# facebookresearch/SONAR

Measured on NVIDIA H100. Metric: sentences/sec->1024-d, higher is better.
Workload: dtype bf16

## Files before the change

include/sonar_b200.h:

```cpp
#ifndef SONAR_B200_H_
#define SONAR_B200_H_

#include <stddef.h>
#include <stdint.h>

#ifdef __cplusplus
extern "C" {
#endif

#define SB_OK 0
#define SB_ERR_INVALID (-1)
#define SB_ERR_CUDA (-2)
#define SB_ERR_DRIVER (-3)
#define SB_ERR_INPUT (-4)

#define SB_POOL_MAX 1
#define SB_POOL_MEAN 2
#define SB_POOL_LAST 3
#define SB_POOL_ATTENTION 4

#define SB_EPI_BIAS 0
#define SB_EPI_BIAS_RELU 1
#define SB_EPI_BIAS_RESIDUAL 2
#define SB_EPI_BIAS_SILU 5
#define SB_EPI_BIAS_TANH 7

typedef struct SbEncoder SbEncoder;

typedef struct SbEncoderConfig {
  int32_t model_dim;
  int32_t num_layers;
  int32_t num_heads;
  int32_t ffn_inner_dim;
  int64_t vocab_size;
  int32_t pos_rows;
  int32_t pooling;
  float ln_eps;
  float embed_scale;
  int32_t cta_group;
  int32_t num_sms;
  int32_t ln_fold;
  int32_t embedding_dim;
  int32_t pooler_layers;
  int32_t pooler_heads;
  int32_t pooler_ffn_inner_dim;
} SbEncoderConfig;

typedef struct SbLayerWeights {
  const void* wqkv;
  const float* bqkv;
  const void* wo;
  const float* bo;
  const void* w1;
  const float* b1;
  const void* w2;
  const float* b2;
  const float* ln1_g;
  const float* ln1_b;
  const float* ln2_g;
  const float* ln2_b;
} SbLayerWeights;

typedef struct SbEncoderWeights {
  const void* embed;
  const float* pos_table;
  const float* final_ln_g;
  const float* final_ln_b;
  const SbLayerWeights* layers;
  const float* pooler_q0;
  const void* proj_w;
  const float* proj_b;
  const struct SbPoolerLayerWeights* pooler;
} SbEncoderWeights;

const char* sb_last_error(void);
int sb_version(void);

int sb_encoder_create(const SbEncoderConfig* cfg, const SbEncoderWeights* w, SbEncoder** out);
void sb_encoder_destroy(SbEncoder* enc);

int sb_encoder_workspace_bytes(const SbEncoder* enc, int32_t max_batch, int64_t max_tokens, size_t* bytes);

int sb_encoder_forward(SbEncoder* enc, const int64_t* ids, int64_t ids_row_stride, const int32_t* seq_lens_host,
                       int32_t batch, int32_t seq_len, float* out, float* encoded, void* workspace,
                       size_t workspace_bytes, void* stream);

int sb_encoder_forward_host(SbEncoder* enc, const int64_t* ids_host, const int32_t* seq_lens_host, int32_t batch,
                            int32_t seq_len, float* out_host, int64_t* ids_staging, float* out_staging,
                            void* workspace, size_t workspace_bytes, void* stream);

int sb_encoder_profile_ffn1(SbEncoder* enc, void* start_event, void* stop_event);

int sb_encoder_check_inputs(SbEncoder* enc, void* workspace, void* stream);


int sb_fold_layernorm(const void* W, const float* bias, const float* gamma, const float* beta, int32_t N, int32_t K,
                      void* Wf, float* colsum, float* bias_f, void* stream);
int sb_gemm_ln_consumer(const void* A, int64_t lda, const void* Wf, int64_t ldw, void* C, int64_t ldc, const float* bias_f,
                        const float* colsum, const float* stats, float eps, int32_t M, int32_t N, int32_t K, int32_t relu,
                        void* stream);
int sb_gemm_residual_stats(const void* A, int64_t lda, const void* W, int64_t ldw, float* x, int64_t ldx, const float* bias,
                           void* h_out, int64_t ldh, float* stats_out, int32_t M, int32_t N, int32_t K, void* stream);

int sb_gemm_residual_splitk(const void* A, int64_t lda, const void* W, int64_t ldw, float* x, int64_t ldx, const float* bias,
                            int32_t M, int32_t N, int32_t K, int32_t* counters, int64_t n_counters, void* stream);

int sb_gemm_bf16(const void* A, int64_t lda, const void* W, int64_t ldw, void* C, int64_t ldc, int32_t out_fp32,
                 const float* bias, const void* residual, int64_t ldr, int32_t M, int32_t N, int32_t K, int32_t epi,
                 int32_t cta_group, void* stream);

int sb_layernorm(const float* x, const float* gamma, const float* beta, float eps, void* y, int64_t T, int32_t D,
                 void* stream);

int sb_attention(const void* qkv, const int32_t* cu_seqlens, int32_t B, int32_t H, int64_t total_tokens, void* out,
                 void* stream);

int sb_embed(const int64_t* ids, int64_t ids_row_stride, const int32_t* cu_seqlens, int32_t B, int32_t S,
             const void* embed, int64_t vocab, const float* pos_table, int32_t pos_rows, int32_t D, float scale,
             float* x, int32_t* err_flag, void* stream);

int sb_pool(const float* x, const int32_t* cu_seqlens, int32_t B, int32_t D, const float* gamma, const float* beta,
            float eps, int32_t apply_ln, int32_t pool_mode, float* out, float* encoded_padded, int32_t S_padded,
            void* stream);

int sb_pool_latent_attention(const void* qt, const void* mem, const int32_t* cu_seqlens, int32_t B, int32_t Hd, int32_t D,
                             void* u, void* stream);

int sb_attention_relpos(const void* qkv, const void* p, const float* u_bias, const float* v_bias, const int32_t* cu_seqlens,
                        int32_t B, int32_t H, int64_t total_tokens, int32_t Npad, int32_t S_center, int32_t impl, void* qu,
                        void* qv, float* vp, void* out, void* stream);
int sb_conformer_conv(const void* g, const int32_t* cu_seqlens, int32_t B, int32_t max_len, int32_t D, const float* dw,
                      const float* bn_scale, const float* bn_shift, void* out, void* stream);
int sb_speech_frontend(const float* fbank, int32_t padded_frames, const int32_t* cu_seqlens, int32_t B, int32_t max_len,
                       const float* gamma, const float* beta, float eps, void* out, void* stream);

typedef struct SbDecoder SbDecoder;

typedef struct SbDecoderConfig {
  int32_t model_dim;
  int32_t num_layers;
  int32_t num_heads;
  int32_t ffn_inner_dim;
  int32_t input_dim;
  int64_t vocab_size;
  int32_t pos_rows;
  int32_t eos_idx;
  float ln_eps;
  float embed_scale;
} SbDecoderConfig;

typedef struct SbDecoderLayerWeights {
  const void* wqkv;
  const float* bqkv;
  const void* wo;
  const float* bo;
  const void* cross_wv;
  const float* cross_bv;
  const void* cross_wo;
  const float* cross_bo;
  const void* w1;
  const float* b1;
  const void* w2;
  const float* b2;
  const float* ln1_g;
  const float* ln1_b;
  const float* ln3_g;
  const float* ln3_b;
} SbDecoderLayerWeights;

typedef struct SbDecoderWeights {
  const void* embed;
  const float* pos_table;
  const float* final_ln_g;
  const float* final_ln_b;
  const SbDecoderLayerWeights* layers;
} SbDecoderWeights;

int sb_decoder_create(const SbDecoderConfig* cfg, const SbDecoderWeights* w, SbDecoder** out);
void sb_decoder_destroy(SbDecoder* dec);
int sb_decoder_workspace_bytes(const SbDecoder* dec, int32_t num_sentences, int32_t beam, int32_t max_len, size_t* bytes);
int sb_decoder_begin(SbDecoder* dec, const float* embeddings, int32_t num_sentences, int32_t beam, int32_t max_len,
                     void* workspace, size_t workspace_bytes, void* stream);
int sb_decoder_step(SbDecoder* dec, const int64_t* tokens, const int32_t* table, int32_t t, int32_t num_sentences,
                    int32_t beam, int32_t max_len, float* out_lprob, int32_t* out_tok, float* out_eos_lprob,
                    const int64_t* probe_tokens, float* out_probe_lprob, void* workspace, size_t workspace_bytes,
                    void* stream);
int sb_decoder_check_inputs(SbDecoder* dec, void* workspace, void* stream);

size_t sb_fbank_tables_bytes(void);
int sb_fbank_build_tables(void* host_buf);
int sb_fbank(const float* waves, const int64_t* wave_offsets, const int32_t* frame_offsets, int32_t B,
             int32_t total_frames, const void* tables, float* raw_out, float* out, int32_t padded_frames, void* stream);

typedef struct SbSpeechEncoder SbSpeechEncoder;

typedef struct SbSpeechConfig {
  int32_t model_dim;
  int32_t num_layers;
  int32_t num_heads;
  int32_t ffn_inner_dim;
  int32_t conv_kernel;
  int32_t pooler_layers;
  int32_t pooler_ffn_inner_dim;
  float ln_eps;
  int32_t attn_impl;
} SbSpeechConfig;

typedef struct SbConformerLayerWeights {
  const float* ffn1_ln_g; const float* ffn1_ln_b;
  const void* ffn1_w1; const float* ffn1_b1; const void* ffn1_w2 ; const float* ffn1_b2 ;
  const float* attn_ln_g; const float* attn_ln_b;
  const void* wqkv; const float* bqkv; const void* wo; const float* bo;
  const void* wr;
  const float* u_bias;
  const float* v_bias;
  const float* conv_ln_g; const float* conv_ln_b;
  const void* pw1;
  const float* dw;
  const float* bn_scale;
  const float* bn_shift;
  const void* pw2;
  const float* ffn2_ln_g; const float* ffn2_ln_b;
  const void* ffn2_w1; const float* ffn2_b1; const void* ffn2_w2 ; const float* ffn2_b2 ;
  const float* ln_g; const float* ln_b;
} SbConformerLayerWeights;

typedef struct SbPoolerLayerWeights {
  const void* sa_wv; const float* sa_bv; const void* sa_wo; const float* sa_bo;
  const float* sa_ln_g; const float* sa_ln_b;
  const void* ca_wq; const float* ca_bq;
  const void* ca_wkv ; const float* ca_bkv;
  const void* ca_wo; const float* ca_bo;
  const float* ca_ln_g; const float* ca_ln_b;
  const void* w1; const float* b1; const void* w2; const float* b2;
  const float* ffn_ln_g; const float* ffn_ln_b;
} SbPoolerLayerWeights;

typedef struct SbSpeechWeights {
  const float* front_ln_g;
  const float* front_ln_b;
  const void* front_w;
  const float* front_b;
  const float* final_ln_g;
  const float* final_ln_b;
  const float* pooler_q0;
  const void* proj_w;
  const float* zeros;
  const SbConformerLayerWeights* layers;
  const SbPoolerLayerWeights* pooler;
} SbSpeechWeights;

int sb_speech_encoder_create(const SbSpeechConfig* cfg, const SbSpeechWeights* w, SbSpeechEncoder** out);
void sb_speech_encoder_destroy(SbSpeechEncoder* enc);
int sb_speech_encoder_workspace_bytes(const SbSpeechEncoder* enc, int32_t batch, int64_t total_positions,
                                      int32_t max_positions, size_t* bytes);
int sb_speech_encoder_forward(SbSpeechEncoder* enc, const float* fbank, int32_t padded_frames, const int32_t* cu_dev,
                              const int32_t* lens_host, int32_t batch, const void* relpos_table, int32_t relpos_rows,
                              float* out, float* encoded_packed, void* workspace, size_t workspace_bytes, void* stream);


int sb_xsim_workspace_bytes(int32_t n, int32_t m, int32_t d, size_t* bytes);

int sb_xsim_knn(const float* x, const float* y, int32_t n, int32_t m, int32_t d, int32_t k, double* out_val,
                int32_t* out_idx, void* workspace, size_t workspace_bytes, void* stream);

int sb_xsim_bidir_workspace_bytes(int32_t n, int32_t m, int32_t d, size_t* bytes);
int sb_xsim_knn_bidir(const float* x, const float* y, int32_t n, int32_t m, int32_t d, int32_t k, double* val_xy,
                      int32_t* idx_xy, double* val_yx, int32_t* idx_yx, int32_t* overflow_flag, void* workspace,
                      size_t workspace_bytes, void* stream);

int sb_xsim_margin_predict(const double* val_xy, const int32_t* idx_xy, const double* val_yx, int32_t n, int32_t m,
                           int32_t k, int32_t margin_mode, int32_t* pred, void* stream);

int sb_beam_step(const float* lp, const int32_t* tok, const float* eos_lp, int64_t* seqs, int32_t* table,
                 int64_t* tokens, float* cum, uint8_t* alive, uint8_t* done, float* fin_score, int64_t* fin_seq,
                 int64_t* fin_len, int64_t* fin_count, int32_t N, int32_t beam, int32_t Tmax, int32_t t, int32_t g,
                 int32_t eos_block, int32_t max_gen, int64_t vocab, int32_t eos, int32_t unk, int32_t pad,
                 float unk_penalty, float score_div, int32_t normalize, void* stream);

typedef struct SbLaser2 SbLaser2;

typedef struct SbLaser2Config {
  int64_t vocab_size;
  int64_t pad_idx;
  int32_t embed_dim;
  int32_t hidden_size;
  int32_t num_layers;
  int32_t bidirectional;
  float padding_value;
  int32_t num_sms;
} SbLaser2Config;

typedef struct SbLstmLayerWeights {
  const void* w_ih;
  const void* w_hh;
  const float* b_ih;
  const float* b_hh;
} SbLstmLayerWeights;

typedef struct SbLaser2Weights {
  const void* embed;
  const SbLstmLayerWeights* layers;
} SbLaser2Weights;

int sb_laser2_create(const SbLaser2Config* cfg, const SbLaser2Weights* w, SbLaser2** out);
void sb_laser2_destroy(SbLaser2* enc);
int sb_laser2_workspace_bytes(const SbLaser2* enc, int32_t max_batch, int64_t max_tokens, size_t* bytes);
int sb_laser2_forward(SbLaser2* enc, const int64_t* ids, int64_t ids_row_stride, const int32_t* seq_lens_host, int32_t batch,
                      int32_t seq_len, float* out, void* workspace, size_t workspace_bytes, void* stream);
int sb_laser2_check_inputs(SbLaser2* enc, void* stream);

int sb_lstm_recurrent(const void* G, int64_t ldg, const void* w_hh, const int32_t* cu_seqlens, const int32_t* tile_seqs,
                      int32_t num_tiles, int32_t num_dirs, void* y, int64_t ldy, float* pool_out, int64_t ldp,
                      const uint8_t* pad_mask, const uint8_t* tail_keep, float padding_value, void* stream);

#define SB_BLASER_COMET 0
#define SB_BLASER_QE 1

typedef struct SbBlaser SbBlaser;

typedef struct SbBlaserConfig {
  int32_t input_form;
  int32_t embedding_dim;
  int32_t num_hidden;
  const int32_t* hidden_dims;
  int32_t cta_group;
  int32_t num_sms;
} SbBlaserConfig;

typedef struct SbBlaserWeights {
  const void* const* w;
  const float* const* b;
} SbBlaserWeights;

int sb_blaser_create(const SbBlaserConfig* cfg, const SbBlaserWeights* w, SbBlaser** out);
void sb_blaser_destroy(SbBlaser* model);
int sb_blaser_workspace_bytes(const SbBlaser* model, int32_t max_rows, size_t* bytes);
int sb_blaser_forward(SbBlaser* model, const float* src, const float* mt, const float* ref, int64_t ld, int32_t rows,
                      float* scores, void* workspace, size_t workspace_bytes, void* stream);
int sb_blaser_featurize(const float* src, const float* mt, const float* ref, int64_t ld, int32_t rows, int32_t E,
                        int32_t input_form, int32_t normalize, void* out, int32_t out_fp32, void* stream);

#ifdef __cplusplus
}
#endif
#endif
```

sonar_b200/_lib.py:

```python

from __future__ import annotations

import ctypes as C
from pathlib import Path
from typing import Optional

_LIB_PATH = Path(__file__).resolve().parent / "lib" / "libsonar_b200.so"
_lib: Optional[C.CDLL] = None

SB_POOL_MAX, SB_POOL_MEAN, SB_POOL_LAST, SB_POOL_ATTENTION = 1, 2, 3, 4
SB_EPI_BIAS, SB_EPI_BIAS_RELU, SB_EPI_BIAS_RESIDUAL, SB_EPI_BIAS_TANH = 0, 1, 2, 7
SB_BLASER_COMET, SB_BLASER_QE = 0, 1
SB_ERR_INVALID, SB_ERR_CUDA, SB_ERR_DRIVER, SB_ERR_INPUT = -1, -2, -3, -4


class SbEncoderConfig(C.Structure):
    _fields_ = [
        ("model_dim", C.c_int32), ("num_layers", C.c_int32), ("num_heads", C.c_int32),
        ("ffn_inner_dim", C.c_int32), ("vocab_size", C.c_int64), ("pos_rows", C.c_int32),
        ("pooling", C.c_int32), ("ln_eps", C.c_float), ("embed_scale", C.c_float),
        ("cta_group", C.c_int32), ("num_sms", C.c_int32), ("ln_fold", C.c_int32),
        ("embedding_dim", C.c_int32), ("pooler_layers", C.c_int32), ("pooler_heads", C.c_int32),
        ("pooler_ffn_inner_dim", C.c_int32),
    ]


class SbLayerWeights(C.Structure):
    _fields_ = [(n, C.c_void_p) for n in (
        "wqkv", "bqkv", "wo", "bo", "w1", "b1", "w2", "b2", "ln1_g", "ln1_b", "ln2_g", "ln2_b")]


class SbPoolerLayerWeights(C.Structure):
    _fields_ = [(n, C.c_void_p) for n in (
        "sa_wv", "sa_bv", "sa_wo", "sa_bo", "sa_ln_g", "sa_ln_b", "ca_wq", "ca_bq", "ca_wkv", "ca_bkv", "ca_wo", "ca_bo",
        "ca_ln_g", "ca_ln_b", "w1", "b1", "w2", "b2", "ffn_ln_g", "ffn_ln_b")]


class SbEncoderWeights(C.Structure):
    _fields_ = [("embed", C.c_void_p), ("pos_table", C.c_void_p), ("final_ln_g", C.c_void_p),
                ("final_ln_b", C.c_void_p), ("layers", C.POINTER(SbLayerWeights)),
                ("pooler_q0", C.c_void_p), ("proj_w", C.c_void_p), ("proj_b", C.c_void_p),
                ("pooler", C.POINTER(SbPoolerLayerWeights))]


class SbDecoderConfig(C.Structure):
    _fields_ = [
        ("model_dim", C.c_int32), ("num_layers", C.c_int32), ("num_heads", C.c_int32),
        ("ffn_inner_dim", C.c_int32), ("input_dim", C.c_int32), ("vocab_size", C.c_int64),
        ("pos_rows", C.c_int32), ("eos_idx", C.c_int32), ("ln_eps", C.c_float), ("embed_scale", C.c_float),
    ]


class SbDecoderLayerWeights(C.Structure):
    _fields_ = [(n, C.c_void_p) for n in (
        "wqkv", "bqkv", "wo", "bo", "cross_wv", "cross_bv", "cross_wo", "cross_bo", "w1", "b1", "w2", "b2",
        "ln1_g", "ln1_b", "ln3_g", "ln3_b")]


class SbDecoderWeights(C.Structure):
    _fields_ = [("embed", C.c_void_p), ("pos_table", C.c_void_p), ("final_ln_g", C.c_void_p),
                ("final_ln_b", C.c_void_p), ("layers", C.POINTER(SbDecoderLayerWeights))]


class SbSpeechConfig(C.Structure):
    _fields_ = [("model_dim", C.c_int32), ("num_layers", C.c_int32), ("num_heads", C.c_int32),
                ("ffn_inner_dim", C.c_int32), ("conv_kernel", C.c_int32), ("pooler_layers", C.c_int32),
                ("pooler_ffn_inner_dim", C.c_int32), ("ln_eps", C.c_float), ("attn_impl", C.c_int32)]


class SbConformerLayerWeights(C.Structure):
    _fields_ = [(n, C.c_void_p) for n in (
        "ffn1_ln_g", "ffn1_ln_b", "ffn1_w1", "ffn1_b1", "ffn1_w2", "ffn1_b2", "attn_ln_g", "attn_ln_b", "wqkv", "bqkv",
        "wo", "bo", "wr", "u_bias", "v_bias", "conv_ln_g", "conv_ln_b", "pw1", "dw", "bn_scale", "bn_shift", "pw2",
        "ffn2_ln_g", "ffn2_ln_b", "ffn2_w1", "ffn2_b1", "ffn2_w2", "ffn2_b2", "ln_g", "ln_b")]


class SbSpeechWeights(C.Structure):
    _fields_ = [(n, C.c_void_p) for n in ("front_ln_g", "front_ln_b", "front_w", "front_b", "final_ln_g", "final_ln_b",
                                          "pooler_q0", "proj_w", "zeros")] + \
               [("layers", C.POINTER(SbConformerLayerWeights)), ("pooler", C.POINTER(SbPoolerLayerWeights))]


class SbLaser2Config(C.Structure):
    _fields_ = [("vocab_size", C.c_int64), ("pad_idx", C.c_int64), ("embed_dim", C.c_int32), ("hidden_size", C.c_int32),
                ("num_layers", C.c_int32), ("bidirectional", C.c_int32), ("padding_value", C.c_float),
                ("num_sms", C.c_int32)]


class SbLstmLayerWeights(C.Structure):
    _fields_ = [(n, C.c_void_p) for n in ("w_ih", "w_hh", "b_ih", "b_hh")]


class SbLaser2Weights(C.Structure):
    _fields_ = [("embed", C.c_void_p), ("layers", C.POINTER(SbLstmLayerWeights))]


class SbBlaserConfig(C.Structure):
    _fields_ = [("input_form", C.c_int32), ("embedding_dim", C.c_int32), ("num_hidden", C.c_int32),
                ("hidden_dims", C.POINTER(C.c_int32)), ("cta_group", C.c_int32), ("num_sms", C.c_int32)]


class SbBlaserWeights(C.Structure):
    _fields_ = [("w", C.POINTER(C.c_void_p)), ("b", C.POINTER(C.c_void_p))]


_SIGNATURES = {
    "sb_last_error": (C.c_char_p, []),
    "sb_version": (C.c_int, []),
    "sb_encoder_create": (C.c_int, [C.POINTER(SbEncoderConfig), C.POINTER(SbEncoderWeights),
                                    C.POINTER(C.c_void_p)]),
    "sb_encoder_destroy": (None, [C.c_void_p]),
    "sb_encoder_workspace_bytes": (C.c_int, [C.c_void_p, C.c_int32, C.c_int64, C.POINTER(C.c_size_t)]),
    "sb_encoder_forward": (C.c_int, [C.c_void_p, C.c_void_p, C.c_int64, C.c_void_p, C.c_int32, C.c_int32,
                                     C.c_void_p, C.c_void_p, C.c_void_p, C.c_size_t, C.c_void_p]),
    "sb_encoder_forward_host": (C.c_int, [C.c_void_p, C.c_void_p, C.c_void_p, C.c_int32, C.c_int32,
                                          C.c_void_p, C.c_void_p, C.c_void_p, C.c_void_p, C.c_size_t,
                                          C.c_void_p]),
    "sb_encoder_profile_ffn1": (C.c_int, [C.c_void_p, C.c_void_p, C.c_void_p]),
    "sb_encoder_check_inputs": (C.c_int, [C.c_void_p, C.c_void_p, C.c_void_p]),
    "sb_gemm_bf16": (C.c_int, [C.c_void_p, C.c_int64, C.c_void_p, C.c_int64, C.c_void_p, C.c_int64,
                               C.c_int32, C.c_void_p, C.c_void_p, C.c_int64, C.c_int32, C.c_int32,
                               C.c_int32, C.c_int32, C.c_int32, C.c_void_p]),
    "sb_layernorm": (C.c_int, [C.c_void_p, C.c_void_p, C.c_void_p, C.c_float, C.c_void_p, C.c_int64,
                               C.c_int32, C.c_void_p]),
    "sb_attention": (C.c_int, [C.c_void_p, C.c_void_p, C.c_int32, C.c_int32, C.c_int64, C.c_void_p, C.c_void_p]),
    "sb_embed": (C.c_int, [C.c_void_p, C.c_int64, C.c_void_p, C.c_int32, C.c_int32, C.c_void_p, C.c_int64,
                           C.c_void_p, C.c_int32, C.c_int32, C.c_float, C.c_void_p, C.c_void_p, C.c_void_p]),
    "sb_pool": (C.c_int, [C.c_void_p, C.c_void_p, C.c_int32, C.c_int32, C.c_void_p, C.c_void_p, C.c_float,
                          C.c_int32, C.c_int32, C.c_void_p, C.c_void_p, C.c_int32, C.c_void_p]),
    "sb_pool_latent_attention": (C.c_int, [C.c_void_p, C.c_void_p, C.c_void_p, C.c_int32, C.c_int32, C.c_int32,
                                           C.c_void_p, C.c_void_p]),
    "sb_attention_relpos": (C.c_int, [C.c_void_p] * 5 + [C.c_int32, C.c_int32, C.c_int64, C.c_int32, C.c_int32, C.c_int32] +
                            [C.c_void_p] * 5),
    "sb_conformer_conv": (C.c_int, [C.c_void_p, C.c_void_p, C.c_int32, C.c_int32, C.c_int32] + [C.c_void_p] * 5),
    "sb_speech_frontend": (C.c_int, [C.c_void_p, C.c_int32, C.c_void_p, C.c_int32, C.c_int32, C.c_void_p, C.c_void_p,
                                     C.c_float, C.c_void_p, C.c_void_p]),
    "sb_decoder_create": (C.c_int, [C.POINTER(SbDecoderConfig), C.POINTER(SbDecoderWeights), C.POINTER(C.c_void_p)]),
    "sb_decoder_destroy": (None, [C.c_void_p]),
    "sb_decoder_workspace_bytes": (C.c_int, [C.c_void_p, C.c_int32, C.c_int32, C.c_int32, C.POINTER(C.c_size_t)]),
    "sb_decoder_begin": (C.c_int, [C.c_void_p, C.c_void_p, C.c_int32, C.c_int32, C.c_int32, C.c_void_p, C.c_size_t,
                                   C.c_void_p]),
    "sb_decoder_step": (C.c_int, [C.c_void_p, C.c_void_p, C.c_void_p, C.c_int32, C.c_int32, C.c_int32, C.c_int32,
                                  C.c_void_p, C.c_void_p, C.c_void_p, C.c_void_p, C.c_void_p, C.c_void_p, C.c_size_t,
                                  C.c_void_p]),
    "sb_decoder_check_inputs": (C.c_int, [C.c_void_p, C.c_void_p, C.c_void_p]),
    "sb_fbank_tables_bytes": (C.c_size_t, []),
    "sb_fbank_build_tables": (C.c_int, [C.c_void_p]),
    "sb_fbank": (C.c_int, [C.c_void_p, C.c_void_p, C.c_void_p, C.c_int32, C.c_int32, C.c_void_p, C.c_void_p,
                           C.c_void_p, C.c_int32, C.c_void_p]),
    "sb_speech_encoder_create": (C.c_int, [C.POINTER(SbSpeechConfig), C.POINTER(SbSpeechWeights), C.POINTER(C.c_void_p)]),
    "sb_speech_encoder_destroy": (None, [C.c_void_p]),
    "sb_speech_encoder_workspace_bytes": (C.c_int, [C.c_void_p, C.c_int32, C.c_int64, C.c_int32, C.POINTER(C.c_size_t)]),
    "sb_speech_encoder_forward": (C.c_int, [C.c_void_p, C.c_void_p, C.c_int32, C.c_void_p, C.c_void_p, C.c_int32,
                                            C.c_void_p, C.c_int32, C.c_void_p, C.c_void_p, C.c_void_p, C.c_size_t,
                                            C.c_void_p]),
    "sb_xsim_workspace_bytes": (C.c_int, [C.c_int32, C.c_int32, C.c_int32, C.POINTER(C.c_size_t)]),
    "sb_xsim_knn": (C.c_int, [C.c_void_p, C.c_void_p, C.c_int32, C.c_int32, C.c_int32, C.c_int32, C.c_void_p,
                              C.c_void_p, C.c_void_p, C.c_size_t, C.c_void_p]),
    "sb_xsim_margin_predict": (C.c_int, [C.c_void_p, C.c_void_p, C.c_void_p, C.c_int32, C.c_int32, C.c_int32,
                                         C.c_int32, C.c_void_p, C.c_void_p]),
    "sb_fold_layernorm": (C.c_int, [C.c_void_p] * 4 + [C.c_int32, C.c_int32] + [C.c_void_p] * 4),
    "sb_gemm_ln_consumer": (C.c_int, [C.c_void_p, C.c_int64, C.c_void_p, C.c_int64, C.c_void_p, C.c_int64, C.c_void_p,
                                      C.c_void_p, C.c_void_p, C.c_float, C.c_int32, C.c_int32, C.c_int32, C.c_int32,
                                      C.c_void_p]),
    "sb_gemm_residual_stats": (C.c_int, [C.c_void_p, C.c_int64, C.c_void_p, C.c_int64, C.c_void_p, C.c_int64, C.c_void_p,
                                         C.c_void_p, C.c_int64, C.c_void_p, C.c_int32, C.c_int32, C.c_int32, C.c_void_p]),
    "sb_gemm_residual_splitk": (C.c_int, [C.c_void_p, C.c_int64, C.c_void_p, C.c_int64, C.c_void_p, C.c_int64, C.c_void_p,
                                          C.c_int32, C.c_int32, C.c_int32, C.c_void_p, C.c_int64, C.c_void_p]),
    "sb_xsim_bidir_workspace_bytes": (C.c_int, [C.c_int32, C.c_int32, C.c_int32, C.POINTER(C.c_size_t)]),
    "sb_xsim_knn_bidir": (C.c_int, [C.c_void_p, C.c_void_p, C.c_int32, C.c_int32, C.c_int32, C.c_int32, C.c_void_p, C.c_void_p,
                                    C.c_void_p, C.c_void_p, C.c_void_p, C.c_void_p, C.c_size_t, C.c_void_p]),
    "sb_beam_step": (C.c_int, [C.c_void_p] * 13 + [C.c_int32] * 7 + [C.c_int64] + [C.c_int32] * 3 +
                     [C.c_float, C.c_float, C.c_int32, C.c_void_p]),
    "sb_laser2_create": (C.c_int, [C.POINTER(SbLaser2Config), C.POINTER(SbLaser2Weights), C.POINTER(C.c_void_p)]),
    "sb_laser2_destroy": (None, [C.c_void_p]),
    "sb_laser2_workspace_bytes": (C.c_int, [C.c_void_p, C.c_int32, C.c_int64, C.POINTER(C.c_size_t)]),
    "sb_laser2_forward": (C.c_int, [C.c_void_p, C.c_void_p, C.c_int64, C.c_void_p, C.c_int32, C.c_int32, C.c_void_p,
                                    C.c_void_p, C.c_size_t, C.c_void_p]),
    "sb_laser2_check_inputs": (C.c_int, [C.c_void_p, C.c_void_p]),
    "sb_lstm_recurrent": (C.c_int, [C.c_void_p, C.c_int64, C.c_void_p, C.c_void_p, C.c_void_p, C.c_int32, C.c_int32,
                                    C.c_void_p, C.c_int64, C.c_void_p, C.c_int64, C.c_void_p, C.c_void_p, C.c_float,
                                    C.c_void_p]),
    "sb_blaser_create": (C.c_int, [C.POINTER(SbBlaserConfig), C.POINTER(SbBlaserWeights), C.POINTER(C.c_void_p)]),
    "sb_blaser_destroy": (None, [C.c_void_p]),
    "sb_blaser_workspace_bytes": (C.c_int, [C.c_void_p, C.c_int32, C.POINTER(C.c_size_t)]),
    "sb_blaser_forward": (C.c_int, [C.c_void_p, C.c_void_p, C.c_void_p, C.c_void_p, C.c_int64, C.c_int32, C.c_void_p,
                                    C.c_void_p, C.c_size_t, C.c_void_p]),
    "sb_blaser_featurize": (C.c_int, [C.c_void_p, C.c_void_p, C.c_void_p, C.c_int64, C.c_int32, C.c_int32, C.c_int32,
                                      C.c_int32, C.c_void_p, C.c_int32, C.c_void_p]),
}


def lib_path() -> Path:
    return _LIB_PATH


def load() -> C.CDLL:
    global _lib
    if _lib is not None:
        return _lib
    if not _LIB_PATH.exists():
        raise RuntimeError(
            f"sonar_b200: native library {_LIB_PATH} is missing -- run `python -m sonar_b200.build` "
            "(or `__graft_entry__.build()`); there is no CPU/PyTorch fallback path.")
    lib = C.CDLL(str(_LIB_PATH))
    for name, (restype, argtypes) in _SIGNATURES.items():
        fn = getattr(lib, name)
        fn.restype = restype
        fn.argtypes = argtypes
    _lib = lib
    return lib


def last_error() -> str:
    msg = load().sb_last_error()
    return msg.decode("utf-8", "replace") if msg else ""


def workspace_bytes(query, *args) -> int:
    need = C.c_size_t()
    check(query(*args, C.byref(need)), query.__name__)
    return need.value


def check(rc: int, what: str) -> None:
    if rc == 0:
        return
    msg = f"{what}: {last_error()} (code {rc})"
    if rc in (SB_ERR_INVALID, SB_ERR_INPUT):
        raise ValueError(msg)
    raise RuntimeError(msg)
```

sonar_b200/csrc/common.cuh:

```cuda
#pragma once

#include <cuda.h>
#include <cuda_bf16.h>
#include <cuda_runtime.h>
#include <stdint.h>
#include <stdio.h>

namespace sb {

void set_last_error(const char* fmt, ...);

#define SB_CUDA_CHECK(expr)                                                              \
  do {                                                                                   \
    cudaError_t _e = (expr);                                                             \
    if (_e != cudaSuccess) {                                                             \
      ::sb::set_last_error("%s failed: %s (%s:%d)", #expr, cudaGetErrorString(_e),       \
                           __FILE__, __LINE__);                                          \
      return -2;                                                                         \
    }                                                                                    \
  } while (0)

__device__ __forceinline__ uint32_t smem_u32(const void* p) {
  return static_cast<uint32_t>(__cvta_generic_to_shared(p));
}

__device__ __forceinline__ uint32_t lane_id() {
  uint32_t l;
  asm volatile("mov.u32 %0, %%laneid;" : "=r"(l));
  return l;
}

__device__ __forceinline__ uint32_t cluster_ctarank() {
  uint32_t r;
  asm volatile("mov.u32 %0, %%cluster_ctarank;" : "=r"(r));
  return r;
}

__device__ __forceinline__ bool elect_one() {
  uint32_t pred = 0;
  asm volatile(
      "{\n\t"
      ".reg .pred p;\n\t"
      "elect.sync _|p, 0xffffffff;\n\t"
      "selp.u32 %0, 1, 0, p;\n\t"
      "}\n"
      : "=r"(pred));
  return pred != 0;
}

__device__ __forceinline__ void cluster_sync_all() {
  asm volatile("barrier.cluster.arrive.release.aligned;\n\t"
               "barrier.cluster.wait.acquire.aligned;\n" ::: "memory");
}

__device__ __forceinline__ void named_bar_sync(uint32_t id, uint32_t nthreads) {
  asm volatile("bar.sync %0, %1;" ::"r"(id), "r"(nthreads) : "memory");
}

__device__ __forceinline__ void mbar_init(uint64_t* bar, uint32_t count) {
  asm volatile("mbarrier.init.shared::cta.b64 [%0], %1;" ::"r"(smem_u32(bar)), "r"(count) : "memory");
}

__device__ __forceinline__ void fence_mbar_init() {
  asm volatile("fence.mbarrier_init.release.cluster;" ::: "memory");
}

__device__ __forceinline__ void mbar_arrive_expect_tx(uint64_t* bar, uint32_t bytes) {
  asm volatile("mbarrier.arrive.expect_tx.shared::cta.b64 _, [%0], %1;" ::"r"(smem_u32(bar)), "r"(bytes)
               : "memory");
}

__device__ __forceinline__ void mbar_arrive(uint64_t* bar) {
  asm volatile("mbarrier.arrive.shared::cta.b64 _, [%0];" ::"r"(smem_u32(bar)) : "memory");
}

__device__ __forceinline__ void mbar_arrive_cluster(uint64_t* bar, uint32_t cta) {
  asm volatile(
      "{\n\t"
      ".reg .b32 ra;\n\t"
      "mapa.shared::cluster.u32 ra, %0, %1;\n\t"
      "mbarrier.arrive.shared::cluster.b64 _, [ra];\n\t"
      "}\n" ::"r"(smem_u32(bar)),
      "r"(cta)
      : "memory");
}

__device__ __forceinline__ bool mbar_try_wait(uint64_t* bar, uint32_t parity) {
  uint32_t ok;
  asm volatile(
      "{\n\t"
      ".reg .pred p;\n\t"
      "mbarrier.try_wait.parity.shared::cta.b64 p, [%1], %2;\n\t"
      "selp.u32 %0, 1, 0, p;\n\t"
      "}\n"
      : "=r"(ok)
      : "r"(smem_u32(bar)), "r"(parity)
      : "memory");
  return ok != 0;
}

__device__ __forceinline__ bool mbar_test_wait(uint64_t* bar, uint32_t parity) {
  uint32_t ok;
  asm volatile(
      "{\n\t"
      ".reg .pred p;\n\t"
      "mbarrier.test_wait.parity.shared::cta.b64 p, [%1], %2;\n\t"
      "selp.u32 %0, 1, 0, p;\n\t"
      "}\n"
      : "=r"(ok)
      : "r"(smem_u32(bar)), "r"(parity)
      : "memory");
  return ok != 0;
}

#ifndef SB_MBAR_TIMEOUT_CYCLES
#define SB_MBAR_TIMEOUT_CYCLES (4000000000ll)
#endif
__device__ __forceinline__ void mbar_wait(uint64_t* bar, uint32_t parity) {
  if (mbar_try_wait(bar, parity)) return;
  const long long t0 = clock64();
  while (!mbar_try_wait(bar, parity)) {
    if (clock64() - t0 > SB_MBAR_TIMEOUT_CYCLES) __trap();
  }
}

__device__ __forceinline__ void tma_prefetch_desc(const CUtensorMap* m) {
  asm volatile("prefetch.tensormap [%0];" ::"l"(reinterpret_cast<uint64_t>(m)) : "memory");
}

__device__ __forceinline__ void tma_load_2d(void* smem_dst, const CUtensorMap* m, uint64_t* bar, int c0,
                                            int c1) {
  asm volatile(
      "cp.async.bulk.tensor.2d.shared::cluster.global.mbarrier::complete_tx::bytes [%0], [%1, {%3, %4}], [%2];" ::"r"(
          smem_u32(smem_dst)),
      "l"(reinterpret_cast<uint64_t>(m)), "r"(smem_u32(bar)), "r"(c0), "r"(c1)
      : "memory");
}

__device__ __forceinline__ void tma_load_2d_multicast(void* smem_dst, const CUtensorMap* m, uint64_t* bar, int c0, int c1,
                                                      uint16_t cta_mask) {
  asm volatile(
      "cp.async.bulk.tensor.2d.shared::cluster.global.mbarrier::complete_tx::bytes.multicast::cluster [%0], [%1, {%3, "
      "%4}], [%2], %5;" ::"r"(smem_u32(smem_dst)),
      "l"(reinterpret_cast<uint64_t>(m)), "r"(smem_u32(bar)), "r"(c0), "r"(c1), "h"(cta_mask)
      : "memory");
}

__device__ __forceinline__ void tma_store_2d(const CUtensorMap* m, const void* smem_src, int c0, int c1) {
  asm volatile("cp.async.bulk.tensor.2d.global.shared::cta.bulk_group [%0, {%2, %3}], [%1];" ::"l"(
                   reinterpret_cast<uint64_t>(m)),
               "r"(smem_u32(smem_src)), "r"(c0), "r"(c1)
               : "memory");
}

__device__ __forceinline__ void tma_reduce_add_2d(const CUtensorMap* m, const void* smem_src, int c0, int c1) {
  asm volatile("cp.reduce.async.bulk.tensor.2d.global.shared::cta.add.bulk_group [%0, {%2, %3}], [%1];" ::"l"(
                   reinterpret_cast<uint64_t>(m)),
               "r"(smem_u32(smem_src)), "r"(c0), "r"(c1)
               : "memory");
}

__device__ __forceinline__ void tma_store_commit() { asm volatile("cp.async.bulk.commit_group;" ::: "memory"); }

template <int N>
__device__ __forceinline__ void tma_store_wait_read() {
  asm volatile("cp.async.bulk.wait_group.read %0;" ::"n"(N) : "memory");
}

template <int N>
__device__ __forceinline__ void tma_store_wait_all() {
  asm volatile("cp.async.bulk.wait_group %0;" ::"n"(N) : "memory");
}

__device__ __forceinline__ void fence_proxy_async_all() { asm volatile("fence.proxy.async;" ::: "memory"); }
__device__ __forceinline__ int ld_acquire_gpu(const int* p) {
  int v;
  asm volatile("ld.acquire.gpu.global.s32 %0, [%1];" : "=r"(v) : "l"(p) : "memory");
  return v;
}
__device__ __forceinline__ void st_release_gpu(int* p, int v) {
  asm volatile("st.release.gpu.global.s32 [%0], %1;" ::"l"(p), "r"(v) : "memory");
}

__device__ __forceinline__ void fence_proxy_async_smem() {
  asm volatile("fence.proxy.async.shared::cta;" ::: "memory");
}

__device__ __forceinline__ void stmatrix_x4(uint32_t smem_addr, uint32_t r0, uint32_t r1, uint32_t r2, uint32_t r3) {
  asm volatile("stmatrix.sync.aligned.m8n8.x4.shared.b16 [%0], {%1, %2, %3, %4};" ::"r"(smem_addr), "r"(r0), "r"(r1),
               "r"(r2), "r"(r3)
               : "memory");
}

__device__ __forceinline__ void st_shared_v2(uint32_t smem_addr, float x, float y) {
  asm volatile("st.shared.v2.f32 [%0], {%1, %2};" ::"r"(smem_addr), "f"(x), "f"(y) : "memory");
}

__device__ __forceinline__ void wgmma_fence() { asm volatile("wgmma.fence.sync.aligned;" ::: "memory"); }
__device__ __forceinline__ void wgmma_commit() { asm volatile("wgmma.commit_group.sync.aligned;" ::: "memory"); }
template <int N>
__device__ __forceinline__ void wgmma_wait() {
  asm volatile("wgmma.wait_group.sync.aligned %0;" ::"n"(N) : "memory");
}
template <int N>
__device__ __forceinline__ void wgmma_fence_regs(float (&d)[N]) {
#pragma unroll
  for (int i = 0; i < N; ++i) asm volatile("" : "+f"(d[i])::"memory");
}

template <int kRegs>
__device__ __forceinline__ void setmaxnreg_inc() {
  asm volatile("setmaxnreg.inc.sync.aligned.u32 %0;" ::"n"(kRegs));
}
template <int kRegs>
__device__ __forceinline__ void setmaxnreg_dec() {
  asm volatile("setmaxnreg.dec.sync.aligned.u32 %0;" ::"n"(kRegs));
}

__device__ __forceinline__ uint64_t wgmma_desc_kmajor_sw128(uint32_t smem_addr) {
  return uint64_t((smem_addr >> 4) & 0x3FFFu)
         | (uint64_t(1024u >> 4) << 32)
         | (uint64_t(1) << 62);
}
__device__ __forceinline__ uint64_t wgmma_desc_mnmajor_sw128(uint32_t smem_addr) {
  return uint64_t((smem_addr >> 4) & 0x3FFFu) | (uint64_t(1) << 16) | (uint64_t(1024u >> 4) << 32) | (uint64_t(1) << 62);
}

__device__ __forceinline__ void wgmma_m64n256k16_ss(float (&d)[128], uint64_t a_desc, uint64_t b_desc, uint32_t accumulate) {
  asm volatile(
      "{\n\t"
      ".reg .pred p;\n\t"
      "setp.ne.b32 p, %130, 0;\n\t"
      "wgmma.mma_async.sync.aligned.m64n256k16.f32.bf16.bf16 {"
      "%0, %1, %2, %3, %4, %5, %6, %7, %8, %9, %10, %11, %12, %13, %14, %15, %16, %17, %18, %19, %20, %21, %22, %23, "
      "%24, %25, %26, %27, %28, %29, %30, %31, %32, %33, %34, %35, %36, %37, %38, %39, %40, %41, %42, %43, %44, %45, "
      "%46, %47, %48, %49, %50, %51, %52, %53, %54, %55, %56, %57, %58, %59, %60, %61, %62, %63, %64, %65, %66, %67, "
      "%68, %69, %70, %71, %72, %73, %74, %75, %76, %77, %78, %79, %80, %81, %82, %83, %84, %85, %86, %87, %88, %89, "
      "%90, %91, %92, %93, %94, %95, %96, %97, %98, %99, %100, %101, %102, %103, %104, %105, %106, %107, %108, %109, "
      "%110, %111, %112, %113, %114, %115, %116, %117, %118, %119, %120, %121, %122, %123, %124, %125, %126, %127"
      "}, %128, %129, p, 1, 1, 0, 0;\n\t"
      "}\n"
      : "+f"(d[0]), "+f"(d[1]), "+f"(d[2]), "+f"(d[3]), "+f"(d[4]), "+f"(d[5]), "+f"(d[6]), "+f"(d[7]),
        "+f"(d[8]), "+f"(d[9]), "+f"(d[10]), "+f"(d[11]), "+f"(d[12]), "+f"(d[13]), "+f"(d[14]), "+f"(d[15]),
        "+f"(d[16]), "+f"(d[17]), "+f"(d[18]), "+f"(d[19]), "+f"(d[20]), "+f"(d[21]), "+f"(d[22]), "+f"(d[23]),
        "+f"(d[24]), "+f"(d[25]), "+f"(d[26]), "+f"(d[27]), "+f"(d[28]), "+f"(d[29]), "+f"(d[30]), "+f"(d[31]),
        "+f"(d[32]), "+f"(d[33]), "+f"(d[34]), "+f"(d[35]), "+f"(d[36]), "+f"(d[37]), "+f"(d[38]), "+f"(d[39]),
        "+f"(d[40]), "+f"(d[41]), "+f"(d[42]), "+f"(d[43]), "+f"(d[44]), "+f"(d[45]), "+f"(d[46]), "+f"(d[47]),
        "+f"(d[48]), "+f"(d[49]), "+f"(d[50]), "+f"(d[51]), "+f"(d[52]), "+f"(d[53]), "+f"(d[54]), "+f"(d[55]),
        "+f"(d[56]), "+f"(d[57]), "+f"(d[58]), "+f"(d[59]), "+f"(d[60]), "+f"(d[61]), "+f"(d[62]), "+f"(d[63]),
        "+f"(d[64]), "+f"(d[65]), "+f"(d[66]), "+f"(d[67]), "+f"(d[68]), "+f"(d[69]), "+f"(d[70]), "+f"(d[71]),
        "+f"(d[72]), "+f"(d[73]), "+f"(d[74]), "+f"(d[75]), "+f"(d[76]), "+f"(d[77]), "+f"(d[78]), "+f"(d[79]),
        "+f"(d[80]), "+f"(d[81]), "+f"(d[82]), "+f"(d[83]), "+f"(d[84]), "+f"(d[85]), "+f"(d[86]), "+f"(d[87]),
        "+f"(d[88]), "+f"(d[89]), "+f"(d[90]), "+f"(d[91]), "+f"(d[92]), "+f"(d[93]), "+f"(d[94]), "+f"(d[95]),
        "+f"(d[96]), "+f"(d[97]), "+f"(d[98]), "+f"(d[99]), "+f"(d[100]), "+f"(d[101]), "+f"(d[102]), "+f"(d[103]),
        "+f"(d[104]), "+f"(d[105]), "+f"(d[106]), "+f"(d[107]), "+f"(d[108]), "+f"(d[109]), "+f"(d[110]), "+f"(d[111]),
        "+f"(d[112]), "+f"(d[113]), "+f"(d[114]), "+f"(d[115]), "+f"(d[116]), "+f"(d[117]), "+f"(d[118]), "+f"(d[119]),
        "+f"(d[120]), "+f"(d[121]), "+f"(d[122]), "+f"(d[123]), "+f"(d[124]), "+f"(d[125]), "+f"(d[126]), "+f"(d[127])
      : "l"(a_desc), "l"(b_desc), "r"(accumulate));
}

__device__ __forceinline__ void wgmma_m64n128k16_ss(float (&d)[64], uint64_t a_desc, uint64_t b_desc, uint32_t accumulate) {
  asm volatile(
      "{\n\t"
      ".reg .pred p;\n\t"
      "setp.ne.b32 p, %66, 0;\n\t"
      "wgmma.mma_async.sync.aligned.m64n128k16.f32.bf16.bf16 {"
      "%0, %1, %2, %3, %4, %5, %6, %7, %8, %9, %10, %11, %12, %13, %14, %15, %16, %17, %18, %19, %20, %21, %22, %23, "
      "%24, %25, %26, %27, %28, %29, %30, %31, %32, %33, %34, %35, %36, %37, %38, %39, %40, %41, %42, %43, %44, %45, "
      "%46, %47, %48, %49, %50, %51, %52, %53, %54, %55, %56, %57, %58, %59, %60, %61, %62, %63"
      "}, %64, %65, p, 1, 1, 0, 0;\n\t"
      "}\n"
      : "+f"(d[0]), "+f"(d[1]), "+f"(d[2]), "+f"(d[3]), "+f"(d[4]), "+f"(d[5]), "+f"(d[6]), "+f"(d[7]),
        "+f"(d[8]), "+f"(d[9]), "+f"(d[10]), "+f"(d[11]), "+f"(d[12]), "+f"(d[13]), "+f"(d[14]), "+f"(d[15]),
        "+f"(d[16]), "+f"(d[17]), "+f"(d[18]), "+f"(d[19]), "+f"(d[20]), "+f"(d[21]), "+f"(d[22]), "+f"(d[23]),
        "+f"(d[24]), "+f"(d[25]), "+f"(d[26]), "+f"(d[27]), "+f"(d[28]), "+f"(d[29]), "+f"(d[30]), "+f"(d[31]),
        "+f"(d[32]), "+f"(d[33]), "+f"(d[34]), "+f"(d[35]), "+f"(d[36]), "+f"(d[37]), "+f"(d[38]), "+f"(d[39]),
        "+f"(d[40]), "+f"(d[41]), "+f"(d[42]), "+f"(d[43]), "+f"(d[44]), "+f"(d[45]), "+f"(d[46]), "+f"(d[47]),
        "+f"(d[48]), "+f"(d[49]), "+f"(d[50]), "+f"(d[51]), "+f"(d[52]), "+f"(d[53]), "+f"(d[54]), "+f"(d[55]),
        "+f"(d[56]), "+f"(d[57]), "+f"(d[58]), "+f"(d[59]), "+f"(d[60]), "+f"(d[61]), "+f"(d[62]), "+f"(d[63])
      : "l"(a_desc), "l"(b_desc), "r"(accumulate));
}

__device__ __forceinline__ void wgmma_m64n96k16_ss(float (&d)[48], uint64_t a_desc, uint64_t b_desc, uint32_t accumulate) {
  asm volatile(
      "{\n\t"
      ".reg .pred p;\n\t"
      "setp.ne.b32 p, %50, 0;\n\t"
      "wgmma.mma_async.sync.aligned.m64n96k16.f32.bf16.bf16 {"
      "%0, %1, %2, %3, %4, %5, %6, %7, %8, %9, %10, %11, %12, %13, %14, %15, %16, %17, %18, %19, %20, %21, %22, %23, "
      "%24, %25, %26, %27, %28, %29, %30, %31, %32, %33, %34, %35, %36, %37, %38, %39, %40, %41, %42, %43, %44, %45, "
      "%46, %47"
      "}, %48, %49, p, 1, 1, 0, 0;\n\t"
      "}\n"
      : "+f"(d[0]), "+f"(d[1]), "+f"(d[2]), "+f"(d[3]), "+f"(d[4]), "+f"(d[5]), "+f"(d[6]), "+f"(d[7]),
        "+f"(d[8]), "+f"(d[9]), "+f"(d[10]), "+f"(d[11]), "+f"(d[12]), "+f"(d[13]), "+f"(d[14]), "+f"(d[15]),
        "+f"(d[16]), "+f"(d[17]), "+f"(d[18]), "+f"(d[19]), "+f"(d[20]), "+f"(d[21]), "+f"(d[22]), "+f"(d[23]),
        "+f"(d[24]), "+f"(d[25]), "+f"(d[26]), "+f"(d[27]), "+f"(d[28]), "+f"(d[29]), "+f"(d[30]), "+f"(d[31]),
        "+f"(d[32]), "+f"(d[33]), "+f"(d[34]), "+f"(d[35]), "+f"(d[36]), "+f"(d[37]), "+f"(d[38]), "+f"(d[39]),
        "+f"(d[40]), "+f"(d[41]), "+f"(d[42]), "+f"(d[43]), "+f"(d[44]), "+f"(d[45]), "+f"(d[46]), "+f"(d[47])
      : "l"(a_desc), "l"(b_desc), "r"(accumulate));
}

__device__ __forceinline__ void wgmma_m64n64k16_rs_bt(float (&d)[32], const uint32_t (&a)[4], uint64_t b_desc, uint32_t accumulate) {
  asm volatile(
      "{\n\t"
      ".reg .pred p;\n\t"
      "setp.ne.b32 p, %37, 0;\n\t"
      "wgmma.mma_async.sync.aligned.m64n64k16.f32.bf16.bf16 {"
      "%0, %1, %2, %3, %4, %5, %6, %7, %8, %9, %10, %11, %12, %13, %14, %15, %16, %17, %18, %19, %20, %21, %22, %23, "
      "%24, %25, %26, %27, %28, %29, %30, %31"
      "}, {%32, %33, %34, %35}, %36, p, 1, 1, 1;\n\t"
      "}\n"
      : "+f"(d[0]), "+f"(d[1]), "+f"(d[2]), "+f"(d[3]), "+f"(d[4]), "+f"(d[5]), "+f"(d[6]), "+f"(d[7]),
        "+f"(d[8]), "+f"(d[9]), "+f"(d[10]), "+f"(d[11]), "+f"(d[12]), "+f"(d[13]), "+f"(d[14]), "+f"(d[15]),
        "+f"(d[16]), "+f"(d[17]), "+f"(d[18]), "+f"(d[19]), "+f"(d[20]), "+f"(d[21]), "+f"(d[22]), "+f"(d[23]),
        "+f"(d[24]), "+f"(d[25]), "+f"(d[26]), "+f"(d[27]), "+f"(d[28]), "+f"(d[29]), "+f"(d[30]), "+f"(d[31])
      : "r"(a[0]), "r"(a[1]), "r"(a[2]), "r"(a[3]), "l"(b_desc), "r"(accumulate));
}

__device__ __forceinline__ void mma_m16n8k16_bf16(float (&d)[4], const uint32_t (&a)[4], uint32_t b0, uint32_t b1) {
  asm volatile("mma.sync.aligned.m16n8k16.row.col.f32.bf16.bf16.f32 {%0,%1,%2,%3}, {%4,%5,%6,%7}, {%8,%9}, {%0,%1,%2,%3};"
               : "+f"(d[0]), "+f"(d[1]), "+f"(d[2]), "+f"(d[3])
               : "r"(a[0]), "r"(a[1]), "r"(a[2]), "r"(a[3]), "r"(b0), "r"(b1));
}

__device__ __forceinline__ float ex2_approx(float x) {
  float y;
  asm("ex2.approx.ftz.f32 %0, %1;" : "=f"(y) : "f"(x));
  return y;
}

__device__ __forceinline__ uint32_t pack_bf16x2(float lo, float hi) {
  __nv_bfloat162 v = __floats2bfloat162_rn(lo, hi);
  return *reinterpret_cast<uint32_t*>(&v);
}

__device__ __forceinline__ float warp_sum(float v) {
#pragma unroll
  for (int o = 16; o > 0; o >>= 1) v += __shfl_xor_sync(0xffffffffu, v, o);
  return v;
}
__device__ __forceinline__ float warp_max(float v) {
#pragma unroll
  for (int o = 16; o > 0; o >>= 1) v = fmaxf(v, __shfl_xor_sync(0xffffffffu, v, o));
  return v;
}

}

namespace sb {
static constexpr int kMaxVec = 8;

template <bool kL2 = false>
__device__ __forceinline__ void load_row(const float* row, int nvec, int lane, float4 (&v)[kMaxVec]) {
#pragma unroll
  for (int i = 0; i < kMaxVec; ++i)
    if (i < nvec) v[i] = kL2 ? __ldcg(reinterpret_cast<const float4*>(row + (i * 32 + lane) * 4))
                        : *reinterpret_cast<const float4*>(row + (i * 32 + lane) * 4);
}

__device__ __forceinline__ void normalize_row(float4 (&v)[kMaxVec], int nvec, int lane, int D,
                                              const float* __restrict__ gamma, const float* __restrict__ beta,
                                              float eps) {
  float s = 0.f;
#pragma unroll
  for (int i = 0; i < kMaxVec; ++i)
    if (i < nvec) s += (v[i].x + v[i].y) + (v[i].z + v[i].w);
  const float mean = warp_sum(s) / float(D);
  float q = 0.f;
#pragma unroll
  for (int i = 0; i < kMaxVec; ++i)
    if (i < nvec) {
      const float a = v[i].x - mean, b = v[i].y - mean, c = v[i].z - mean, d = v[i].w - mean;
      q += (a * a + b * b) + (c * c + d * d);
    }
  const float rstd = 1.0f / sqrtf(warp_sum(q) / float(D) + eps);
#pragma unroll
  for (int i = 0; i < kMaxVec; ++i)
    if (i < nvec) {
      const float4 g = __ldg(reinterpret_cast<const float4*>(gamma) + i * 32 + lane);
      const float4 bt = __ldg(reinterpret_cast<const float4*>(beta) + i * 32 + lane);
      v[i].x = (v[i].x - mean) * rstd * g.x + bt.x;
      v[i].y = (v[i].y - mean) * rstd * g.y + bt.y;
      v[i].z = (v[i].z - mean) * rstd * g.z + bt.z;
      v[i].w = (v[i].w - mean) * rstd * g.w + bt.w;
    }
}

}

__device__ __forceinline__ float tanh_approx(float x) {
  float y;
  asm("tanh.approx.f32 %0, %1;" : "=f"(y) : "f"(x));
  return y;
}
__device__ __forceinline__ float sigmoid_fast(float x) { return fmaf(0.5f, tanh_approx(0.5f * x), 0.5f); }
__device__ __forceinline__ float silu_fast(float x) {
  const float h = 0.5f * x;
  return fmaf(h, tanh_approx(h), h);
}
```

sonar_b200/csrc/encoder.cu:

```cuda

#include "../../include/sonar_b200.h"
#include <stdlib.h>

#include "common.cuh"
#include "sonar_b200_internal.h"

#include <cstdarg>
#include <cstdio>
#include <cstring>
#include <new>
#include <vector>

namespace sb {

static thread_local char g_err[512] = "";

void set_last_error(const char* fmt, ...) {
  va_list ap;
  va_start(ap, fmt);
  vsnprintf(g_err, sizeof(g_err), fmt, ap);
  va_end(ap);
}

int require_hopper(const char* who, int* num_sms) {
  int n_gpu = 0, dev = 0, major = 0, minor = 0;
  if (cudaGetDeviceCount(&n_gpu) != cudaSuccess || n_gpu == 0) {
    set_last_error("%s: no CUDA device (this engine has no CPU path)", who);
    return SB_ERR_CUDA;
  }
  SB_CUDA_CHECK(cudaGetDevice(&dev));
  SB_CUDA_CHECK(cudaDeviceGetAttribute(&major, cudaDevAttrComputeCapabilityMajor, dev));
  SB_CUDA_CHECK(cudaDeviceGetAttribute(&minor, cudaDevAttrComputeCapabilityMinor, dev));
  if (major != 9) {
    set_last_error("%s: the sm_90a kernels need a Hopper H100-class GPU (found sm_%d%d)", who, major, minor);
    return SB_ERR_CUDA;
  }
  SB_CUDA_CHECK(cudaDeviceGetAttribute(num_sms, cudaDevAttrMultiProcessorCount, dev));
  return SB_OK;
}

struct Workspace {
  int32_t* cu;
  float* ln_stats;
  float* x;
  __nv_bfloat16* h;
  __nv_bfloat16* qkv;
  __nv_bfloat16* f;
  AttentionPooler::Ws pool;
  size_t bytes;
};

}

using namespace sb;

struct FoldedLayer {
  __nv_bfloat16* wqkv = nullptr;
  __nv_bfloat16* w1 = nullptr;
  float* cqkv = nullptr;
  float* bqkv = nullptr;
  float* c1 = nullptr;
  float* b1 = nullptr;
};

struct SbEncoder {
  SbEncoderConfig cfg;
  int out_dim;
  std::vector<FoldedLayer> folded;
  void* fold_pool = nullptr;
  int32_t* err_flag = nullptr;
  const void* embed;
  const float* pos_table;
  const float* final_ln_g;
  const float* final_ln_b;
  std::vector<SbLayerWeights> layers;
  AttentionPooler pooler;
  int num_sms;
  static constexpr int kSlots = 8;
  static constexpr int kSlotInts = 32768 + 8;
  int32_t* pinned = nullptr;
  cudaEvent_t ev[kSlots];
  bool ev_ok[kSlots];
  unsigned next_slot = 0;
  cudaEvent_t prof_start = nullptr, prof_stop = nullptr;
};

static Workspace carve(const SbEncoder* e, int32_t max_batch, int64_t max_tokens, void* base) {
  const size_t D = e->cfg.model_dim, F = e->cfg.ffn_inner_dim;
  const size_t T = (size_t)(max_tokens > 0 ? max_tokens : 1);
  Carver c(base);
  Workspace w;
  w.cu = c.take<int32_t>(sizeof(int32_t) * ((size_t)max_batch + 1));
  w.ln_stats = c.take<float>(T * (D / kLnPartCols) * 2 * sizeof(float));
  w.x = c.take<float>(T * D * 4);
  w.h = c.take<__nv_bfloat16>(T * D * 2);
  w.qkv = c.take<__nv_bfloat16>(T * 3 * D * 2);
  w.f = c.take<__nv_bfloat16>(T * F * 2);
  w.pool = {};
  if (e->cfg.pooling == SB_POOL_ATTENTION) w.pool = e->pooler.take(c, (size_t)max_batch);
  w.bytes = c.off;
  return w;
}

extern "C" {

const char* sb_last_error(void) { return g_err; }
int sb_version(void) { return 109; }

int sb_encoder_create(const SbEncoderConfig* cfg, const SbEncoderWeights* w, SbEncoder** out) {
  if (!cfg || !w || !out) { set_last_error("sb_encoder_create: null argument"); return SB_ERR_INVALID; }
  *out = nullptr;
  const int D = cfg->model_dim, H = cfg->num_heads, F = cfg->ffn_inner_dim;
  if (D <= 0 || D % 256 != 0 || D > 1024) {
    set_last_error("sb_encoder_create: model_dim must be a multiple of 256 and <= 1024 (got %d)", D);
    return SB_ERR_INVALID;
  }
  if (H <= 0 || D != H * 64) {
    set_last_error("sb_encoder_create: head_dim must be 64 (model_dim=%d, num_heads=%d)", D, H);
    return SB_ERR_INVALID;
  }
  if (F <= 0 || F % 256 != 0) { set_last_error("sb_encoder_create: ffn_inner_dim must be a multiple of 256"); return SB_ERR_INVALID; }
  if (cfg->ln_fold < 0 || cfg->ln_fold > 2) { set_last_error("sb_encoder_create: ln_fold must be 0, 1 or 2"); return SB_ERR_INVALID; }
  if (cfg->num_layers < 0 || cfg->pos_rows <= 0 || cfg->vocab_size <= 0) {
    set_last_error("sb_encoder_create: bad num_layers / pos_rows / vocab_size");
    return SB_ERR_INVALID;
  }
  const bool attn_pool = cfg->pooling == SB_POOL_ATTENTION;
  if (cfg->pooling != SB_POOL_MAX && cfg->pooling != SB_POOL_MEAN && cfg->pooling != SB_POOL_LAST && !attn_pool) {
    set_last_error("sb_encoder_create: unsupported pooling %d", cfg->pooling);
    return SB_ERR_INVALID;
  }
  const int E = cfg->embedding_dim;
  if (attn_pool) {
    if (E <= 0 || E % 256 != 0 || E > 1024 || E != 64 * cfg->pooler_heads) {
      set_last_error("sb_encoder_create: attention pooling needs embedding_dim = 64 * pooler_heads, a multiple of 256 and "
                     "<= 1024 (embedding_dim=%d, pooler_heads=%d)", E, cfg->pooler_heads);
      return SB_ERR_INVALID;
    }
    if (cfg->pooler_ffn_inner_dim <= 0 || cfg->pooler_ffn_inner_dim % 256 != 0 || cfg->pooler_layers < 1) {
      set_last_error("sb_encoder_create: attention pooling needs pooler_layers >= 1 and pooler_ffn_inner_dim a multiple of 256 "
                     "(got %d, %d)", cfg->pooler_layers, cfg->pooler_ffn_inner_dim);
      return SB_ERR_INVALID;
    }
  } else if (E != 0 && E != D) {
    set_last_error("sb_encoder_create: embedding_dim (%d) != model_dim (%d) needs attention pooling", E, D);
    return SB_ERR_INVALID;
  }
  if (!w->embed || !w->pos_table || !w->final_ln_g || !w->final_ln_b || (cfg->num_layers > 0 && !w->layers)) {
    set_last_error("sb_encoder_create: missing weight pointer");
    return SB_ERR_INVALID;
  }
  for (int i = 0; i < cfg->num_layers; ++i)
    if (has_null_pointer(w->layers[i])) {
      set_last_error("sb_encoder_create: layer %d has a null weight pointer", i);
      return SB_ERR_INVALID;
    }
  int num_sms = 0;
  if (int rc = require_hopper("sb_encoder_create", &num_sms)) return rc;
  SbEncoder* e = new (std::nothrow) SbEncoder();
  if (!e) { set_last_error("out of host memory"); return SB_ERR_INVALID; }
  e->cfg = *cfg;
  e->embed = w->embed;
  e->pos_table = w->pos_table;
  e->final_ln_g = w->final_ln_g;
  e->final_ln_b = w->final_ln_b;
  e->layers.assign(w->layers, w->layers + cfg->num_layers);
  e->out_dim = attn_pool ? E : D;
  e->num_sms = cfg->num_sms > 0 ? cfg->num_sms : num_sms;
  for (int i = 0; i < SbEncoder::kSlots; ++i) e->ev_ok[i] = false;
  if (cudaMallocHost(reinterpret_cast<void**>(&e->pinned), sizeof(int32_t) * SbEncoder::kSlots * SbEncoder::kSlotInts) !=
      cudaSuccess) {
    set_last_error("sb_encoder_create: cudaMallocHost failed");
    delete e;
    return SB_ERR_CUDA;
  }
  if (cudaMalloc(reinterpret_cast<void**>(&e->err_flag), 256) != cudaSuccess ||
      cudaMemset(e->err_flag, 0, 256) != cudaSuccess) {
    set_last_error("sb_encoder_create: cudaMalloc of the input-check flag failed");
    sb_encoder_destroy(e);
    return SB_ERR_CUDA;
  }
  if (cfg->ln_fold && cfg->num_layers > 0) {
    const size_t D_ = D, F_ = F;
    auto carve_folded = [&](void* base) {
      Carver c(base);
      for (FoldedLayer& f : e->folded) {
        f.wqkv = c.take<__nv_bfloat16>(3 * D_ * D_ * 2, 256);
        f.w1 = c.take<__nv_bfloat16>(F_ * D_ * 2, 256);
        f.cqkv = c.take<float>(3 * D_ * 4, 256);
        f.bqkv = c.take<float>(3 * D_ * 4, 256);
        f.c1 = c.take<float>(F_ * 4, 256);
        f.b1 = c.take<float>(F_ * 4, 256);
      }
      return c.off;
    };
    e->folded.resize(cfg->num_layers);
    const size_t pool_bytes = carve_folded(nullptr);
    if (cudaMalloc(&e->fold_pool, pool_bytes) != cudaSuccess) {
      set_last_error("sb_encoder_create: cudaMalloc of %zu bytes for the LayerNorm-folded weights failed", pool_bytes);
      sb_encoder_destroy(e);
      return SB_ERR_CUDA;
    }
    carve_folded(e->fold_pool);
    for (int i = 0; i < cfg->num_layers; ++i) {
      const FoldedLayer& f = e->folded[i];
      const SbLayerWeights& l = e->layers[i];
      int rc = fold_layernorm_weights(reinterpret_cast<const __nv_bfloat16*>(l.wqkv), l.bqkv, l.ln1_g, l.ln1_b, 3 * D, D,
                                      f.wqkv, f.cqkv, f.bqkv, nullptr);
      if (!rc)
        rc = fold_layernorm_weights(reinterpret_cast<const __nv_bfloat16*>(l.w1), l.b1, l.ln2_g, l.ln2_b, F, D, f.w1, f.c1,
                                    f.b1, nullptr);
      if (rc) { sb_encoder_destroy(e); return rc; }
    }
    if (cudaDeviceSynchronize() != cudaSuccess) {
      set_last_error("sb_encoder_create: folding the LayerNorm weights failed: %s", cudaGetErrorString(cudaGetLastError()));
      sb_encoder_destroy(e);
      return SB_ERR_CUDA;
    }
  }
  if (attn_pool) {
    const int rc = e->pooler.create("sb_encoder_create", w->pooler, cfg->pooler_layers, w->pooler_q0, w->proj_w, w->proj_b,
                                    D, E, cfg->pooler_ffn_inner_dim, cfg->ln_eps, e->num_sms, cfg->cta_group == 1 ? 1 : 2, 0);
    if (rc) { sb_encoder_destroy(e); return rc; }
  }
  for (int i = 0; i < SbEncoder::kSlots; ++i) {
    if (cudaEventCreateWithFlags(&e->ev[i], cudaEventDisableTiming) != cudaSuccess) {
      set_last_error("sb_encoder_create: cudaEventCreate failed");
      sb_encoder_destroy(e);
      return SB_ERR_CUDA;
    }
    e->ev_ok[i] = true;
  }
  *out = e;
  return SB_OK;
}

void sb_encoder_destroy(SbEncoder* e) {
  if (!e) return;
  for (int i = 0; i < SbEncoder::kSlots; ++i)
    if (e->ev_ok[i]) cudaEventDestroy(e->ev[i]);
  if (e->pinned) cudaFreeHost(e->pinned);
  if (e->fold_pool) cudaFree(e->fold_pool);
  e->pooler.destroy();
  if (e->err_flag) cudaFree(e->err_flag);
  delete e;
}

int sb_encoder_workspace_bytes(const SbEncoder* enc, int32_t max_batch, int64_t max_tokens, size_t* bytes) {
  if (!enc || !bytes || max_batch <= 0 || max_tokens <= 0) {
    set_last_error("sb_encoder_workspace_bytes: bad argument");
    return SB_ERR_INVALID;
  }
  *bytes = carve(enc, max_batch, max_tokens, nullptr).bytes + kWorkspaceAlign;
  return SB_OK;
}

int sb_encoder_forward(SbEncoder* e, const int64_t* ids, int64_t ids_row_stride, const int32_t* seq_lens_host,
                       int32_t B, int32_t S, float* out, float* encoded, void* workspace, size_t workspace_bytes,
                       void* stream_v) {
  if (!e || !ids || !out || !workspace) { set_last_error("sb_encoder_forward: null argument"); return SB_ERR_INVALID; }
  if (B <= 0 || S <= 0) { set_last_error("sb_encoder_forward: empty batch (B=%d, S=%d)", B, S); return SB_ERR_INVALID; }
  if (S > e->cfg.pos_rows) {
    set_last_error("sb_encoder_forward: seq_len %d exceeds the encoder's max_seq_len %d", S, e->cfg.pos_rows);
    return SB_ERR_INVALID;
  }
  if (B + 1 > SbEncoder::kSlotInts) { set_last_error("sb_encoder_forward: batch too large (%d)", B); return SB_ERR_INVALID; }
  if (ids_row_stride < S) { set_last_error("sb_encoder_forward: ids_row_stride < seq_len"); return SB_ERR_INVALID; }
  cudaStream_t stream = reinterpret_cast<cudaStream_t>(stream_v);
  const int D = e->cfg.model_dim, F = e->cfg.ffn_inner_dim, H = e->cfg.num_heads;

  const unsigned slot = e->next_slot++ % SbEncoder::kSlots;
  SB_CUDA_CHECK(cudaEventSynchronize(e->ev[slot]));
  int32_t* cu_h = e->pinned + (size_t)slot * SbEncoder::kSlotInts;
  long long T = 0;
  cu_h[0] = 0;
  for (int b = 0; b < B; ++b) {
    const int len = seq_lens_host ? seq_lens_host[b] : S;
    if (len < 0 || len > S) { set_last_error("sb_encoder_forward: seq_lens[%d]=%d outside [0,%d]", b, len, S); return SB_ERR_INVALID; }
    T += len;
    if (T > 0x7fffffffll) { set_last_error("sb_encoder_forward: too many tokens"); return SB_ERR_INVALID; }
    cu_h[b + 1] = (int32_t)T;
  }
  Workspace w;
  int rc = bind_workspace("sb_encoder_forward", workspace, workspace_bytes, &w,
                          [&](void* p) { return carve(e, B, T, p); });
  if (rc) return rc;
  SB_CUDA_CHECK(cudaMemcpyAsync(w.cu, cu_h, sizeof(int32_t) * (B + 1), cudaMemcpyHostToDevice, stream));
  SB_CUDA_CHECK(cudaEventRecord(e->ev[slot], stream));
  const bool attn_pool = e->cfg.pooling == SB_POOL_ATTENTION;
  if (T == 0) {
    if (!attn_pool) {
      SB_CUDA_CHECK(cudaMemsetAsync(out, 0, sizeof(float) * (size_t)B * D, stream));
      return SB_OK;
    }
    if (encoded) SB_CUDA_CHECK(cudaMemsetAsync(encoded, 0, sizeof(float) * (size_t)B * S * D, stream));
    return e->pooler.forward(w.pool, w.h, w.cu, B, out, stream);
  }

  const bool fold = e->cfg.ln_fold != 0 && e->cfg.num_layers > 0;
  const bool fold2 = fold && e->cfg.ln_fold == 1;
  __nv_bfloat16* hn = w.qkv;
  if ((rc = embed_tokens(ids, ids_row_stride, w.cu, B, S, reinterpret_cast<const __nv_bfloat16*>(e->embed),
                         e->cfg.vocab_size, e->pos_table, e->cfg.pos_rows, D, e->cfg.embed_scale, w.x, e->err_flag,
                         stream, 0, fold ? w.h : nullptr, fold ? w.ln_stats : nullptr)))
    return rc;

  const int cta_group = (e->cfg.cta_group == 1) ? 1 : 2;
  const int M = (int)T;
  LnFold consume;
  consume.stats_in = w.ln_stats;
  consume.chunks = D / kLnPartCols;
  consume.eps = e->cfg.ln_eps;
  for (int li = 0; li < e->cfg.num_layers; ++li) {
    const SbLayerWeights& L = e->layers[li];
    const FoldedLayer* f = fold ? &e->folded[li] : nullptr;
    if (!fold)
      if ((rc = layernorm_bf16(w.x, L.ln1_g, L.ln1_b, e->cfg.ln_eps, w.h, T, D, stream))) return rc;
    GemmArgs qkv = gemm_args(w.h, D, fold ? f->wqkv : L.wqkv, D, w.qkv, 3 * D, 0, fold ? f->bqkv : L.bqkv, M, 3 * D, D,
                             EPI_BIAS, e->num_sms);
    qkv.cta_group = cta_group;
    if (fold) { qkv.lf = consume; qkv.lf.colsum = f->cqkv; }
    if ((rc = gemm_bf16(qkv, stream))) return rc;
    if ((rc = attention_packed(w.qkv, w.cu, B, H, T, e->num_sms, w.h, stream))) return rc;
    GemmArgs proj = gemm_args(w.h, D, L.wo, D, w.x, D, 1, L.bo, M, D, D, EPI_BIAS_RESIDUAL, e->num_sms);
    proj.cta_group = cta_group;
    if (fold2) {
      proj.epi = EPI_BIAS_RESIDUAL_STATS;
      proj.lf.h_out = hn; proj.lf.ldh = D; proj.lf.stats_out = w.ln_stats;
    }
    if ((rc = gemm_bf16(proj, stream))) return rc;
    if (!fold2)
      if ((rc = layernorm_bf16(w.x, L.ln2_g, L.ln2_b, e->cfg.ln_eps, w.h, T, D, stream))) return rc;
    GemmArgs ffn1 = gemm_args(fold2 ? hn : w.h, D, fold2 ? f->w1 : L.w1, D, w.f, F, 0, fold2 ? f->b1 : L.b1, M, F, D,
                              EPI_BIAS_RELU, e->num_sms);
    ffn1.cta_group = cta_group;
    if (fold2) { ffn1.lf = consume; ffn1.lf.colsum = f->c1; }
    const bool prof = e->prof_start && li == e->cfg.num_layers / 2;
    if (prof) SB_CUDA_CHECK(cudaEventRecord(e->prof_start, stream));
    if ((rc = gemm_bf16(ffn1, stream))) return rc;
    if (prof) SB_CUDA_CHECK(cudaEventRecord(e->prof_stop, stream));
    GemmArgs ffn2 = gemm_args(w.f, F, L.w2, F, w.x, D, 1, L.b2, M, D, F, EPI_BIAS_RESIDUAL, e->num_sms);
    ffn2.cta_group = cta_group;
    if (fold && li + 1 < e->cfg.num_layers) {
      ffn2.epi = EPI_BIAS_RESIDUAL_STATS;
      ffn2.lf.h_out = w.h; ffn2.lf.ldh = D; ffn2.lf.stats_out = w.ln_stats;
    }
    if ((rc = gemm_bf16(ffn2, stream))) return rc;
  }
  if (!attn_pool)
    return ln_pool(w.x, w.cu, B, D, e->final_ln_g, e->final_ln_b, e->cfg.ln_eps, 1, e->cfg.pooling, out, encoded, S,
                   stream);
  if ((rc = layernorm_dual(w.x, e->final_ln_g, e->final_ln_b, e->cfg.ln_eps, w.x, w.h, T, D, stream))) return rc;
  if (encoded)
    if ((rc = ln_pool(w.x, w.cu, B, D, nullptr, nullptr, e->cfg.ln_eps, 0, POOL_LAST, w.pool.px, encoded, S, stream)))
      return rc;
  return e->pooler.forward(w.pool, w.h, w.cu, B, out, stream);
}

int sb_encoder_forward_host(SbEncoder* e, const int64_t* ids_host, const int32_t* seq_lens_host, int32_t B,
                            int32_t S, float* out_host, int64_t* ids_staging, float* out_staging, void* workspace,
                            size_t workspace_bytes, void* stream_v) {
  if (!e || !ids_host || !out_host || !ids_staging || !out_staging) {
    set_last_error("sb_encoder_forward_host: null argument");
    return SB_ERR_INVALID;
  }
  if (B <= 0 || S <= 0) { set_last_error("sb_encoder_forward_host: empty batch"); return SB_ERR_INVALID; }
  cudaStream_t stream = reinterpret_cast<cudaStream_t>(stream_v);
  SB_CUDA_CHECK(cudaMemcpyAsync(ids_staging, ids_host, sizeof(int64_t) * (size_t)B * S, cudaMemcpyHostToDevice, stream));
  int rc = sb_encoder_forward(e, ids_staging, S, seq_lens_host, B, S, out_staging, nullptr, workspace, workspace_bytes,
                              stream_v);
  if (rc) return rc;
  SB_CUDA_CHECK(cudaMemcpyAsync(out_host, out_staging, sizeof(float) * (size_t)B * e->out_dim,
                                cudaMemcpyDeviceToHost, stream));
  SB_CUDA_CHECK(cudaStreamSynchronize(stream));
  return SB_OK;
}

int sb_encoder_profile_ffn1(SbEncoder* e, void* start_event, void* stop_event) {
  if (!e || (!start_event) != (!stop_event)) { set_last_error("sb_encoder_profile_ffn1: bad argument"); return SB_ERR_INVALID; }
  e->prof_start = reinterpret_cast<cudaEvent_t>(start_event);
  e->prof_stop = reinterpret_cast<cudaEvent_t>(stop_event);
  return SB_OK;
}

int sb_encoder_check_inputs(SbEncoder* e, void* workspace, void* stream_v) {
  (void)workspace;
  if (!e) { set_last_error("sb_encoder_check_inputs: null argument"); return SB_ERR_INVALID; }
  cudaStream_t stream = reinterpret_cast<cudaStream_t>(stream_v);
  int32_t flag = 0;
  SB_CUDA_CHECK(cudaMemcpyAsync(&flag, e->err_flag, sizeof(int32_t), cudaMemcpyDeviceToHost, stream));
  SB_CUDA_CHECK(cudaMemsetAsync(e->err_flag, 0, sizeof(int32_t), stream));
  SB_CUDA_CHECK(cudaStreamSynchronize(stream));
  if (flag != 0) {
    set_last_error("token id outside [0, vocab_size) in a batch passed to sb_encoder_forward since the last check");
    return SB_ERR_INPUT;
  }
  return SB_OK;
}

int sb_gemm_bf16(const void* A, int64_t lda, const void* W, int64_t ldw, void* C, int64_t ldc, int32_t out_fp32,
                 const float* bias, const void* residual, int64_t ldr, int32_t M, int32_t N, int32_t K, int32_t epi,
                 int32_t cta_group, void* stream) {
  if (!A || !W || !C) { set_last_error("sb_gemm_bf16: null pointer"); return SB_ERR_INVALID; }
  int sms = 0;
  if (int rc = require_hopper("sb_gemm_bf16", &sms)) return rc;
  GemmArgs g = gemm_args(A, lda, W, ldw, C, ldc, out_fp32, bias, M, N, K, epi, sms);
  g.residual = residual; g.ldr = ldr;
  g.cta_group = cta_group == 1 ? 1 : 2;
  g.allow_skinny = (cta_group == 0);
  return gemm_bf16(g, reinterpret_cast<cudaStream_t>(stream));
}

int sb_fold_layernorm(const void* W, const float* bias, const float* gamma, const float* beta, int32_t N, int32_t K,
                      void* Wf, float* colsum, float* bias_f, void* stream) {
  if (!W || !bias || !gamma || !beta || !Wf || !colsum || !bias_f || N <= 0 || K <= 0) {
    set_last_error("sb_fold_layernorm: bad argument");
    return SB_ERR_INVALID;
  }
  return fold_layernorm_weights(reinterpret_cast<const __nv_bfloat16*>(W), bias, gamma, beta, N, K,
                                reinterpret_cast<__nv_bfloat16*>(Wf), colsum, bias_f, reinterpret_cast<cudaStream_t>(stream));
}

int sb_gemm_ln_consumer(const void* A, int64_t lda, const void* Wf, int64_t ldw, void* C, int64_t ldc, const float* bias_f,
                        const float* colsum, const float* stats, float eps, int32_t M, int32_t N, int32_t K, int32_t relu,
                        void* stream) {
  if (!A || !Wf || !C || !bias_f || !colsum || !stats) { set_last_error("sb_gemm_ln_consumer: null pointer"); return SB_ERR_INVALID; }
  int sms = 0;
  if (int rc = require_hopper("sb_gemm_ln_consumer", &sms)) return rc;
  GemmArgs g = gemm_args(A, lda, Wf, ldw, C, ldc, 0, bias_f, M, N, K, relu ? EPI_BIAS_RELU : EPI_BIAS, sms);
  g.lf.stats_in = stats; g.lf.colsum = colsum; g.lf.chunks = K / kLnPartCols; g.lf.eps = eps;
  return gemm_bf16(g, reinterpret_cast<cudaStream_t>(stream));
}

int sb_gemm_residual_stats(const void* A, int64_t lda, const void* W, int64_t ldw, float* x, int64_t ldx, const float* bias,
                           void* h_out, int64_t ldh, float* stats_out, int32_t M, int32_t N, int32_t K, void* stream) {
  if (!A || !W || !x || !bias || !h_out || !stats_out) { set_last_error("sb_gemm_residual_stats: null pointer"); return SB_ERR_INVALID; }
  int sms = 0;
  if (int rc = require_hopper("sb_gemm_residual_stats", &sms)) return rc;
  GemmArgs g = gemm_args(A, lda, W, ldw, x, ldx, 1, bias, M, N, K, EPI_BIAS_RESIDUAL_STATS, sms);
  g.lf.h_out = reinterpret_cast<__nv_bfloat16*>(h_out); g.lf.ldh = ldh; g.lf.stats_out = stats_out;
  return gemm_bf16(g, reinterpret_cast<cudaStream_t>(stream));
}

int sb_gemm_residual_splitk(const void* A, int64_t lda, const void* W, int64_t ldw, float* x, int64_t ldx, const float* bias,
                            int32_t M, int32_t N, int32_t K, int32_t* counters, int64_t n_counters, void* stream) {
  if (!A || !W || !x || !bias || !counters) { set_last_error("sb_gemm_residual_splitk: null pointer"); return SB_ERR_INVALID; }
  int sms = 0;
  if (int rc = require_hopper("sb_gemm_residual_splitk", &sms)) return rc;
  GemmArgs g = gemm_args(A, lda, W, ldw, x, ldx, 1, bias, M, N, K, EPI_BIAS_RESIDUAL, sms);
  g.splitk_flags = counters;
  g.splitk_flags_len = n_counters;
  return gemm_bf16(g, reinterpret_cast<cudaStream_t>(stream));
}

int sb_layernorm(const float* x, const float* gamma, const float* beta, float eps, void* y, int64_t T, int32_t D,
                 void* stream) {
  if (!x || !gamma || !beta || !y) { set_last_error("sb_layernorm: null pointer"); return SB_ERR_INVALID; }
  return layernorm_bf16(x, gamma, beta, eps, reinterpret_cast<__nv_bfloat16*>(y), T, D,
                        reinterpret_cast<cudaStream_t>(stream));
}

int sb_attention(const void* qkv, const int32_t* cu_seqlens, int32_t B, int32_t H, int64_t total_tokens, void* out,
                 void* stream) {
  if (!qkv || !cu_seqlens || !out) { set_last_error("sb_attention: null pointer"); return SB_ERR_INVALID; }
  int sms = 0;
  if (int rc = require_hopper("sb_attention", &sms)) return rc;
  return attention_packed(reinterpret_cast<const __nv_bfloat16*>(qkv), cu_seqlens, B, H, total_tokens, sms,
                          reinterpret_cast<__nv_bfloat16*>(out), reinterpret_cast<cudaStream_t>(stream));
}

int sb_embed(const int64_t* ids, int64_t ids_row_stride, const int32_t* cu_seqlens, int32_t B, int32_t S,
             const void* embed, int64_t vocab, const float* pos_table, int32_t pos_rows, int32_t D, float scale,
             float* x, int32_t* err_flag, void* stream) {
  if (!ids || !cu_seqlens || !embed || !pos_table || !x || !err_flag) {
    set_last_error("sb_embed: null pointer");
    return SB_ERR_INVALID;
  }
  return embed_tokens(ids, ids_row_stride, cu_seqlens, B, S, reinterpret_cast<const __nv_bfloat16*>(embed), vocab,
                      pos_table, pos_rows, D, scale, x, err_flag, reinterpret_cast<cudaStream_t>(stream));
}

int sb_pool_latent_attention(const void* qt, const void* mem, const int32_t* cu_seqlens, int32_t B, int32_t Hd, int32_t D,
                             void* u, void* stream) {
  if (!qt || !mem || !cu_seqlens || !u) { set_last_error("sb_pool_latent_attention: null pointer"); return SB_ERR_INVALID; }
  int sms = 0;
  if (int rc = require_hopper("sb_pool_latent_attention", &sms)) return rc;
  return pool_latent_attention(reinterpret_cast<const __nv_bfloat16*>(qt), reinterpret_cast<const __nv_bfloat16*>(mem),
                               cu_seqlens, B, Hd, D, reinterpret_cast<__nv_bfloat16*>(u), reinterpret_cast<cudaStream_t>(stream));
}

int sb_pool(const float* x, const int32_t* cu_seqlens, int32_t B, int32_t D, const float* gamma, const float* beta,
            float eps, int32_t apply_ln, int32_t pool_mode, float* out, float* encoded_padded, int32_t S_padded,
            void* stream) {
  if (!x || !cu_seqlens || !out) { set_last_error("sb_pool: null pointer"); return SB_ERR_INVALID; }
  return ln_pool(x, cu_seqlens, B, D, gamma, beta, eps, apply_ln, pool_mode, out, encoded_padded, S_padded,
                 reinterpret_cast<cudaStream_t>(stream));
}

}
```

sonar_b200/csrc/gemm_wgmma.cu:

```cuda

#include "common.cuh"
#include "sonar_b200_internal.h"

#include <math_constants.h>

namespace sb {

constexpr bool epi_row_wise(int epi) { return epi == EPI_BIAS_RESIDUAL_STATS || epi == EPI_TOPK; }

template <int kCtaGroup, int kEpi>
struct GemmCfg {
  static constexpr bool ROW_WISE = epi_row_wise(kEpi);
  static constexpr int BLOCK_M = 128;
  static constexpr int BLOCK_N = 256;
  static constexpr int BLOCK_K = 64;
  static constexpr int LOAD_N = BLOCK_N / kCtaGroup;
  static constexpr int A_BYTES = BLOCK_M * BLOCK_K * 2;
  static constexpr int B_BYTES = BLOCK_N * BLOCK_K * 2;
  static constexpr int STAGES = ROW_WISE ? 3 : 4;
  static constexpr int EPI_GROUPS = 2;
  static constexpr int CD_BYTES = 2 * 64 * 128;
  static constexpr int TRANS_LD = 68;
  static constexpr int TRANS_BYTES = ROW_WISE ? 64 * TRANS_LD * 4 : 0;
  static constexpr int LN_BYTES = 64 * 8;
  static constexpr int BAR_BYTES = 256;
  static constexpr int SMEM_BYTES =
      STAGES * (A_BYTES + B_BYTES) + 2 * (CD_BYTES + TRANS_BYTES + LN_BYTES) + BAR_BYTES + 1024 ;
  static constexpr int THREADS = 384;
  static_assert(SMEM_BYTES <= 232448, "shared memory budget of one sm_90 block");
  static_assert(2 * STAGES * 8 <= BAR_BYTES, "ring barriers");
};

template <bool kSweep>
struct TileSched {
  int num_m_tiles, num_n_tiles, cluster_id, num_clusters, n_chunks, tiles_per_chunk;
  int k_splits = 1;
  int i = 0, j = 0;
  __device__ __forceinline__ bool next(int& m_blk, int& n_blk, int& chunk, bool& first, bool& last) {
    if constexpr (!kSweep) {
      const int item = cluster_id + i * num_clusters;
      ++i;
      const int tiles = num_m_tiles * num_n_tiles;
      if (item >= tiles * k_splits) return false;
      const int tile = (k_splits == 1) ? item : item % tiles;
      chunk = (k_splits == 1) ? 0 : item / tiles;
      m_blk = tile / num_n_tiles;
      n_blk = tile % num_n_tiles;
      first = last = true;
      return true;
    } else {
      for (;;) {
        const int item = cluster_id + i * num_clusters;
        if (item >= num_m_tiles * n_chunks) return false;
        m_blk = item / n_chunks;
        chunk = item % n_chunks;
        const int n_begin = chunk * tiles_per_chunk;
        const int cnt = min(tiles_per_chunk, num_n_tiles - n_begin);
        if (j < cnt) {
          n_blk = n_begin + j;
          first = (j == 0);
          last = (j == cnt - 1);
          ++j;
          return true;
        }
        j = 0;
        ++i;
      }
    }
  }
};

template <int KC>
__device__ __forceinline__ void topk_insert(float (&tv)[KC], int (&ti)[KC], float v, int idx) {
  float cv = v;
  int ci = idx;
#pragma unroll
  for (int p = 0; p < KC; ++p) {
    const bool gt = cv > tv[p];
    const float ov = tv[p];
    const int oi = ti[p];
    tv[p] = gt ? cv : ov;
    ti[p] = gt ? ci : oi;
    cv = gt ? ov : cv;
    ci = gt ? oi : ci;
  }
}


template <int kCtaGroup, int kEpi, typename OutT>
__global__ void __launch_bounds__(GemmCfg<kCtaGroup, kEpi>::THREADS, 1)
gemm_bf16_wgmma_kernel(const __grid_constant__ CUtensorMap tm_a, const __grid_constant__ CUtensorMap tm_b,
                       const __grid_constant__ CUtensorMap tm_c, const float* __restrict__ bias,
                       const OutT* residual, long long ldr, int M, int N, int K, float* __restrict__ cand_val,
                       int* __restrict__ cand_idx, float* __restrict__ lse_part, int n_chunks, const LnFold lf,
                       const ColFilter cf, int k_splits, int* __restrict__ splitk_flags) {
  constexpr bool kSweep = (kEpi == EPI_TOPK);
  using Cfg = GemmCfg<kCtaGroup, kEpi>;
  extern __shared__ uint8_t smem_raw[];
  uint8_t* smem = reinterpret_cast<uint8_t*>((reinterpret_cast<uintptr_t>(smem_raw) + 1023) & ~uintptr_t(1023));
  uint8_t* smem_a = smem;
  uint8_t* smem_b = smem_a + Cfg::STAGES * Cfg::A_BYTES;
  uint8_t* smem_cd = smem_b + Cfg::STAGES * Cfg::B_BYTES;
  uint8_t* smem_tr = smem_cd + 2 * Cfg::CD_BYTES;
  uint8_t* smem_ln = smem_tr + 2 * Cfg::TRANS_BYTES;
  uint64_t* full_bar = reinterpret_cast<uint64_t*>(smem_ln + 2 * Cfg::LN_BYTES);
  uint64_t* empty_bar = full_bar + Cfg::STAGES;

  const int warp_idx = threadIdx.x >> 5;
  const int lane = threadIdx.x & 31;
  const int wg_idx = __shfl_sync(0xffffffffu, threadIdx.x >> 7, 0);
  const uint32_t cta_rank = (kCtaGroup == 2) ? cluster_ctarank() : 0u;

  if (threadIdx.x == 0) {
    tma_prefetch_desc(&tm_a);
    tma_prefetch_desc(&tm_b);
    tma_prefetch_desc(&tm_c);
    for (int i = 0; i < Cfg::STAGES; ++i) {
      mbar_init(&full_bar[i], 1);
      mbar_init(&empty_bar[i], 8 * kCtaGroup);
    }
    fence_mbar_init();
  }
  if (kCtaGroup == 2) cluster_sync_all(); else __syncthreads();

  const int tile_m = Cfg::BLOCK_M * kCtaGroup;
  const int num_m_tiles = (M + tile_m - 1) / tile_m;
  const int num_n_tiles = (N + Cfg::BLOCK_N - 1) / Cfg::BLOCK_N;
  const int num_kb = K / Cfg::BLOCK_K;
  const int cluster_id = blockIdx.x / kCtaGroup;
  const int num_clusters = gridDim.x / kCtaGroup;
  TileSched<kSweep> sched{num_m_tiles, num_n_tiles, cluster_id, num_clusters, n_chunks,
                          (num_n_tiles + n_chunks - 1) / n_chunks, (kEpi == EPI_BIAS_ACCUM) ? k_splits : 1};
  auto kb_begin = [&](int split) { return (kEpi == EPI_BIAS_ACCUM && k_splits > 1) ? split * num_kb / k_splits : 0; };
  auto kb_end = [&](int split) { return (kEpi == EPI_BIAS_ACCUM && k_splits > 1) ? (split + 1) * num_kb / k_splits : num_kb; };
  int m_blk, n_blk, chunk;
  bool first_in_item, last_in_item;

  if (wg_idx == 0) {
    setmaxnreg_dec<40>();
    if (warp_idx == 0 && lane == 0) {
      int stage = 0;
      uint32_t phase = 0;
      while (sched.next(m_blk, n_blk, chunk, first_in_item, last_in_item)) {
        const int m0 = m_blk * tile_m + int(cta_rank) * Cfg::BLOCK_M;
        const int n0 = n_blk * Cfg::BLOCK_N + int(cta_rank) * Cfg::LOAD_N;
        const int kb1 = kb_end(chunk);
        for (int kb = kb_begin(chunk); kb < kb1; ++kb) {
          mbar_wait(&empty_bar[stage], phase ^ 1);
          mbar_arrive_expect_tx(&full_bar[stage], Cfg::A_BYTES + Cfg::B_BYTES);
          tma_load_2d(smem_a + stage * Cfg::A_BYTES, &tm_a, &full_bar[stage], kb * Cfg::BLOCK_K, m0);
          uint8_t* b_dst = smem_b + stage * Cfg::B_BYTES + int(cta_rank) * (Cfg::LOAD_N * Cfg::BLOCK_K * 2);
          if (kCtaGroup == 2) tma_load_2d_multicast(b_dst, &tm_b, &full_bar[stage], kb * Cfg::BLOCK_K, n0, 0x3);
          else tma_load_2d(b_dst, &tm_b, &full_bar[stage], kb * Cfg::BLOCK_K, n0);
          if (++stage == Cfg::STAGES) { stage = 0; phase ^= 1; }
        }
      }
    }
    __syncwarp();
  } else {
    setmaxnreg_inc<232>();
    const int cwg = wg_idx - 1;
    const int t = threadIdx.x & 127;
    const int half = t >> 6;
    const int erow = t & 63;
    const int row_in_tile = cwg * 64 + erow;
    const int frow = (warp_idx & 3) * 16 + (lane >> 2);
    uint8_t* smem_cd_wg = smem_cd + cwg * Cfg::CD_BYTES;
    float* trans = reinterpret_cast<float*>(smem_tr + cwg * Cfg::TRANS_BYTES);
    float2* ln_sm = reinterpret_cast<float2*>(smem_ln + cwg * Cfg::LN_BYTES);
    const uint32_t bar_id = 1 + cwg;
    const uint64_t a_desc0 = wgmma_desc_kmajor_sw128(smem_u32(smem_a) + cwg * 64 * 128);
    const uint64_t b_desc0 = wgmma_desc_kmajor_sw128(smem_u32(smem_b));
    auto release = [&](int stage) {
      if (kCtaGroup == 2) { if (lane < 2) mbar_arrive_cluster(&empty_bar[stage], lane); }
      else if (lane == 0) mbar_arrive(&empty_bar[stage]);
    };
    int stage = 0;
    uint32_t phase = 0;
    float acc[128];
    constexpr int KC = kTopkCandidates;
    [[maybe_unused]] float tv[KC];
    [[maybe_unused]] int ti[KC];
    [[maybe_unused]] float run_max = -CUDART_INF_F, run_sum = 0.f;
    [[maybe_unused]] int q_n = 0;
    [[maybe_unused]] bool fold_in = false;
    [[maybe_unused]] float2 part_next[8];
    [[maybe_unused]] TileSched<kSweep> sched_ahead = sched;
    [[maybe_unused]] auto fetch_parts = [&]() {
      int mb, nb, ch;
      bool f0, f1;
      if (!sched_ahead.next(mb, nb, ch, f0, f1)) return;
      const int r = mb * tile_m + int(cta_rank) * Cfg::BLOCK_M + row_in_tile;
      if (r < M) {
        const float2* sp = reinterpret_cast<const float2*>(lf.stats_in) + (long long)r * lf.chunks;
#pragma unroll
        for (int i = 0; i < 8; ++i)
          if (i < lf.chunks) part_next[i] = sp[i];
      }
    };
    if constexpr (kEpi == EPI_BIAS || kEpi == EPI_BIAS_RELU) {
      fold_in = lf.stats_in != nullptr;
      if (fold_in) fetch_parts();
    }
    while (sched.next(m_blk, n_blk, chunk, first_in_item, last_in_item)) {
      const int m0 = m_blk * tile_m + int(cta_rank) * Cfg::BLOCK_M;
      const int n0 = n_blk * Cfg::BLOCK_N;
      const int grow = m0 + row_in_tile;
      [[maybe_unused]] float ln_mean = 0.f, ln_rstd = 1.f;
      if constexpr (kEpi == EPI_BIAS || kEpi == EPI_BIAS_RELU) {
        if (fold_in) {
          if (grow < M) {
            float msum = 0.f;
#pragma unroll
            for (int i = 0; i < 8; ++i)
              if (i < lf.chunks) msum += part_next[i].x;
            ln_mean = msum / float(lf.chunks);
            float m2 = 0.f;
#pragma unroll
            for (int i = 0; i < 8; ++i)
              if (i < lf.chunks) { const float dm = part_next[i].x - ln_mean; m2 += part_next[i].y + float(kLnPartCols) * dm * dm; }
            ln_rstd = 1.0f / sqrtf(m2 / float(kLnPartCols * lf.chunks) + lf.eps);
          }
          if (half == 0) ln_sm[erow] = make_float2(ln_mean, ln_rstd);
          fetch_parts();
        }
      }
      [[maybe_unused]] float4 rnext[8];
      [[maybe_unused]] float st_n = 0.f, st_mean = 0.f, st_m2 = 0.f;
      if constexpr (kEpi == EPI_BIAS_RESIDUAL_STATS) {
#pragma unroll
        for (int q = 0; q < 8; ++q) rnext[q] = make_float4(0.f, 0.f, 0.f, 0.f);
        if (grow < M) {
          const float4* rp = reinterpret_cast<const float4*>(reinterpret_cast<const float*>(residual) + (long long)grow * ldr +
                                                             n0 + half * 128);
#pragma unroll
          for (int q = 0; q < 8; ++q) rnext[q] = rp[q];
        }
      }
      {
        const int kb0 = kb_begin(chunk), kb1 = kb_end(chunk);
        auto issue = [&](bool first) {
          const uint64_t a_desc = a_desc0 + uint64_t(stage * (Cfg::A_BYTES >> 4));
          const uint64_t b_desc = b_desc0 + uint64_t(stage * (Cfg::B_BYTES >> 4));
          wgmma_fence_regs(acc);
          wgmma_fence();
#pragma unroll
          for (int k = 0; k < Cfg::BLOCK_K / 16; ++k)
            wgmma_m64n256k16_ss(acc, a_desc + uint64_t(2 * k), b_desc + uint64_t(2 * k), (first && k == 0) ? 0u : 1u);
          wgmma_commit();
          wgmma_fence_regs(acc);
        };
        mbar_wait(&full_bar[stage], phase);
        issue(true);
        int prev = stage;
        if (++stage == Cfg::STAGES) { stage = 0; phase ^= 1; }
        for (int kb = kb0 + 1; kb < kb1; ++kb) {
          mbar_wait(&full_bar[stage], phase);
          issue(false);
          wgmma_wait<1>();
          release(prev);
          prev = stage;
          if (++stage == Cfg::STAGES) { stage = 0; phase ^= 1; }
        }
        wgmma_wait<0>();
        wgmma_fence_regs(acc);
        release(prev);
      }
      if constexpr (!Cfg::ROW_WISE) {
        constexpr int BOX_COLS = 128 / int(sizeof(OutT));
        constexpr int BOXES = Cfg::BLOCK_N / BOX_COLS;
        constexpr int BOX_BYTES = 64 * 128;
        constexpr int NBUF = Cfg::CD_BYTES / BOX_BYTES;
        static_assert(NBUF >= 2 && BOXES % NBUF == 0, "staging buffers must alternate the same way in every tile");
        const int fcol = 2 * (lane & 3);
        const int grow_lo = m0 + cwg * 64 + frow, grow_hi = grow_lo + 8;
        if (fold_in) named_bar_sync(bar_id, 128);
        const bool with_bias = !(kEpi == EPI_BIAS_ACCUM && chunk > 0);
        auto epi = [&](float v, float b, float c, float2 ln, int grow, int col) -> float {
          float f = fold_in ? fmaf(ln.y, fmaf(-ln.x, c, v), b) : v + b;
          if constexpr (kEpi == EPI_BIAS_RELU) f = fmaxf(f, 0.0f);
          if constexpr (kEpi == EPI_BIAS_SILU) f = silu_fast(f);
          if constexpr (kEpi == EPI_BIAS_TANH) {
            const float h = 0.5f * f;
            f = tanh_approx(h + h);
          }
          if constexpr (kEpi == EPI_BIAS_RESIDUAL) {
            if (grow < M) {
              if constexpr (sizeof(OutT) == 4) f += reinterpret_cast<const float*>(residual)[(long long)grow * ldr + col];
              else f += __bfloat162float(reinterpret_cast<const __nv_bfloat16*>(residual)[(long long)grow * ldr + col]);
            }
          }
          return f;
        };
        auto group = [&](int j, float (&o)[4]) {
          const int col = n0 + 8 * j + fcol;
          const float2 b2 = with_bias ? __ldg(reinterpret_cast<const float2*>(bias + col)) : make_float2(0.f, 0.f);
          const float2 c2 = fold_in ? __ldg(reinterpret_cast<const float2*>(lf.colsum + col)) : make_float2(0.f, 0.f);
          const float2 ln_lo = fold_in ? ln_sm[frow] : make_float2(0.f, 1.f);
          const float2 ln_hi = fold_in ? ln_sm[frow + 8] : make_float2(0.f, 1.f);
          o[0] = epi(acc[4 * j + 0], b2.x, c2.x, ln_lo, grow_lo, col);
          o[1] = epi(acc[4 * j + 1], b2.y, c2.y, ln_lo, grow_lo, col + 1);
          o[2] = epi(acc[4 * j + 2], b2.x, c2.x, ln_hi, grow_hi, col);
          o[3] = epi(acc[4 * j + 3], b2.y, c2.y, ln_hi, grow_hi, col + 1);
        };
        const uint32_t cd_base = smem_u32(smem_cd_wg);
#pragma unroll
        for (int b = 0; b < BOXES; ++b) {
          const uint32_t buf = cd_base + (b % NBUF) * BOX_BYTES;
          if constexpr (sizeof(OutT) == 2) {
            const int mrow = (warp_idx & 3) * 16 + (lane & 7) + 8 * ((lane >> 3) & 1);
#pragma unroll
            for (int p = 0; p < BOX_COLS / 16; ++p) {
              const int j = b * (BOX_COLS / 8) + 2 * p;
              float o0[4], o1[4];
              group(j, o0);
              group(j + 1, o1);
              const int q = 2 * p + (lane >> 4);
              stmatrix_x4(buf + mrow * 128 + ((q ^ (lane & 7)) << 4), pack_bf16x2(o0[0], o0[1]), pack_bf16x2(o0[2], o0[3]),
                          pack_bf16x2(o1[0], o1[1]), pack_bf16x2(o1[2], o1[3]));
            }
          } else {
#pragma unroll
            for (int jj = 0; jj < BOX_COLS / 8; ++jj) {
              float o[4];
              group(b * (BOX_COLS / 8) + jj, o);
              const int q = 2 * jj + ((lane >> 1) & 1);
              const uint32_t a = buf + frow * 128 + ((q ^ (frow & 7)) << 4) + 8 * (lane & 1);
              st_shared_v2(a, o[0], o[1]);
              st_shared_v2(a + 8 * 128, o[2], o[3]);
            }
          }
          fence_proxy_async_smem();
          if (t == 0) tma_store_wait_read<NBUF - 2>();
          named_bar_sync(bar_id, 128);
          if (t == 0) {
            const int c0 = n0 + b * BOX_COLS, r0 = m0 + cwg * 64;
            if constexpr (kEpi == EPI_BIAS_ACCUM) {
              int* flag = nullptr;
              if (k_splits > 1) {
                flag = splitk_flags + ((long long)(m_blk * num_n_tiles + n_blk) * kCtaGroup + int(cta_rank)) * 2 + cwg;
                if (b == 0 && chunk > 0) {
                  while (ld_acquire_gpu(flag) != chunk) __nanosleep(64);
                  fence_proxy_async_all();
                }
              }
              tma_reduce_add_2d(&tm_c, reinterpret_cast<const void*>(smem_cd_wg + (b % NBUF) * BOX_BYTES), c0, r0);
              tma_store_commit();
              if (k_splits > 1 && b == BOXES - 1) {
                tma_store_wait_all<0>();
                fence_proxy_async_all();
                __threadfence();
                st_release_gpu(flag, chunk == k_splits - 1 ? 0 : chunk + 1);
              }
            } else {
              tma_store_2d(&tm_c, smem_cd_wg + (b % NBUF) * BOX_BYTES, c0, r0);
              tma_store_commit();
            }
          }
        }
        continue;
      }
      auto stage_piece = [&](int s) {
        named_bar_sync(bar_id, 128);
        float* tr = trans + frow * Cfg::TRANS_LD + 2 * (lane & 3);
#pragma unroll
        for (int hh = 0; hh < 2; ++hh)
#pragma unroll
          for (int jj = 0; jj < 4; ++jj) {
            const int j = 16 * hh + 4 * s + jj;
            *reinterpret_cast<float2*>(tr + 32 * hh + 8 * jj) = make_float2(acc[4 * j], acc[4 * j + 1]);
            *reinterpret_cast<float2*>(tr + 8 * Cfg::TRANS_LD + 32 * hh + 8 * jj) = make_float2(acc[4 * j + 2], acc[4 * j + 3]);
          }
        named_bar_sync(bar_id, 128);
      };
      auto load_piece = [&](uint32_t (&v)[32]) {
        const float4* src = reinterpret_cast<const float4*>(trans + erow * Cfg::TRANS_LD + half * 32);
#pragma unroll
        for (int i = 0; i < 8; ++i) {
          const float4 x = src[i];
          v[4 * i] = __float_as_uint(x.x); v[4 * i + 1] = __float_as_uint(x.y);
          v[4 * i + 2] = __float_as_uint(x.z); v[4 * i + 3] = __float_as_uint(x.w);
        }
      };
      if constexpr (kEpi == EPI_TOPK) {
        if (first_in_item) {
#pragma unroll
          for (int p = 0; p < KC; ++p) { tv[p] = -CUDART_INF_F; ti[p] = -1; }
          run_max = -CUDART_INF_F;
          run_sum = 0.f;
        }
        const bool cf_on = cf.thr != nullptr && grow < M;
        constexpr int kQ = 16;
        uint2* queue = reinterpret_cast<uint2*>(smem_cd_wg) + t;
        auto drain = [&]() {
          const int rounds = __reduce_max_sync(0xffffffffu, q_n);
          for (int r = 0; r < rounds; ++r) {
            if (r < q_n) {
              const uint2 e = queue[r * 128];
              const float x = __uint_as_float(e.x);
              if (x > tv[KC - 1]) topk_insert<KC>(tv, ti, x, int(e.y));
            }
          }
          q_n = 0;
        };
#pragma unroll
        for (int s = 0; s < 4; ++s) {
          uint32_t v[32];
          stage_piece(s);
          load_piece(v);
          const int gcol = n0 + half * 128 + s * 32;
          if (gcol + 32 > N) {
#pragma unroll
            for (int j = 0; j < 32; ++j)
              if (gcol + j >= N) v[j] = __float_as_uint(-CUDART_INF_F);
          }
          float gm[4];
#pragma unroll
          for (int g8 = 0; g8 < 4; ++g8) {
            float mx = __uint_as_float(v[g8 * 8]);
#pragma unroll
            for (int j = 1; j < 8; ++j) mx = fmaxf(mx, __uint_as_float(v[g8 * 8 + j]));
            gm[g8] = mx;
          }
          if (lse_part != nullptr) {
            const float cm = fmaxf(fmaxf(gm[0], gm[1]), fmaxf(gm[2], gm[3]));
            if (cm > run_max) {
              run_sum *= __expf(run_max - cm);
              run_max = cm;
            }
            if (run_max > -CUDART_INF_F) {
              float cs = 0.f;
#pragma unroll
              for (int j = 0; j < 32; ++j) cs += __expf(__uint_as_float(v[j]) - run_max);
              run_sum += cs;
            }
          }
          const float thr = tv[KC - 1];
          float t8[4] = {CUDART_INF_F, CUDART_INF_F, CUDART_INF_F, CUDART_INF_F};
          if (cf_on) {
            const float4 tt = __ldg(reinterpret_cast<const float4*>(cf.thr8 + (gcol >> 3)));
            t8[0] = tt.x; t8[1] = tt.y; t8[2] = tt.z; t8[3] = tt.w;
          }
#pragma unroll
          for (int g8 = 0; g8 < 4; ++g8) {
            if (gm[g8] > t8[g8]) {
              const float4 t0 = *reinterpret_cast<const float4*>(cf.thr + gcol + g8 * 8);
              const float4 t1 = *reinterpret_cast<const float4*>(cf.thr + gcol + g8 * 8 + 4);
              const float th[8] = {t0.x, t0.y, t0.z, t0.w, t1.x, t1.y, t1.z, t1.w};
#pragma unroll
              for (int j = 0; j < 8; ++j) {
                const float x = __uint_as_float(v[g8 * 8 + j]);
                if (x > th[j]) {
                  const int col = gcol + g8 * 8 + j;
                  const int slot = atomicAdd(cf.cnt + col, 1);
                  if (slot < cf.cap) cf.buf[(long long)col * cf.cap + slot] = make_uint2(__float_as_uint(x), uint32_t(grow));
                  else cf.thr[col] = CUDART_INF_F;
                }
              }
            }
            if (gm[g8] > thr) {
#pragma unroll
              for (int j = 0; j < 8; ++j) {
                const float x = __uint_as_float(v[g8 * 8 + j]);
                if (x > thr) {
                  queue[q_n * 128] = make_uint2(__float_as_uint(x), uint32_t(gcol + g8 * 8 + j));
                  ++q_n;
                }
              }
            }
            if (__any_sync(0xffffffffu, q_n > kQ - 8)) drain();
          }
        }
        if (last_in_item) drain();
        if (last_in_item && grow < M) {
          const long long slot = ((long long)grow * n_chunks + chunk) * Cfg::EPI_GROUPS + half;
#pragma unroll
          for (int p = 0; p < KC; ++p) {
            cand_val[slot * KC + p] = tv[p];
            cand_idx[slot * KC + p] = ti[p];
          }
          if (lse_part != nullptr) {
            lse_part[slot * 2] = run_max;
            lse_part[slot * 2 + 1] = run_sum;
          }
        }
        continue;
      }
      if constexpr (kEpi == EPI_BIAS_RESIDUAL_STATS) {
#pragma unroll
        for (int s = 0; s < 4; ++s) {
          if (t == 0) tma_store_wait_read<0>();
          uint32_t v[32];
          stage_piece(s);
          load_piece(v);
          uint8_t* cd_row = smem_cd_wg + half * (64 * 128) + erow * 128;
          const int gcol = n0 + half * 128 + s * 32;
          float f[32];
#pragma unroll
          for (int j = 0; j < 32; j += 4) {
            const float4 b4 = __ldg(reinterpret_cast<const float4*>(bias + gcol + j));
            f[j + 0] = __uint_as_float(v[j + 0]) + b4.x;
            f[j + 1] = __uint_as_float(v[j + 1]) + b4.y;
            f[j + 2] = __uint_as_float(v[j + 2]) + b4.z;
            f[j + 3] = __uint_as_float(v[j + 3]) + b4.w;
          }
          float4 rcur[8];
#pragma unroll
          for (int q = 0; q < 8; ++q) rcur[q] = rnext[q];
          if (s + 1 < 4 && grow < M) {
            const float4* rp = reinterpret_cast<const float4*>(reinterpret_cast<const float*>(residual) +
                                                               (long long)grow * ldr + gcol + 32);
#pragma unroll
            for (int q = 0; q < 8; ++q) rnext[q] = rp[q];
          }
#pragma unroll
          for (int q = 0; q < 8; ++q) {
            f[4 * q + 0] += rcur[q].x; f[4 * q + 1] += rcur[q].y; f[4 * q + 2] += rcur[q].z; f[4 * q + 3] += rcur[q].w;
          }
          float cs = 0.f;
#pragma unroll
          for (int j = 0; j < 32; ++j) cs += f[j];
          const float cm = cs * (1.0f / 32.0f);
          float cq = 0.f;
#pragma unroll
          for (int j = 0; j < 32; ++j) { const float dv = f[j] - cm; cq = fmaf(dv, dv, cq); }
          const float n_new = st_n + 32.f;
          const float dlt = cm - st_mean;
          st_mean = fmaf(dlt, 32.f / n_new, st_mean);
          st_m2 += cq + dlt * dlt * (st_n * 32.f / n_new);
          st_n = n_new;
          if (grow < M) {
            uint4* hp = reinterpret_cast<uint4*>(lf.h_out + (long long)grow * lf.ldh + gcol);
#pragma unroll
            for (int q = 0; q < 4; ++q)
              hp[q] = make_uint4(pack_bf16x2(f[8 * q], f[8 * q + 1]), pack_bf16x2(f[8 * q + 2], f[8 * q + 3]),
                                 pack_bf16x2(f[8 * q + 4], f[8 * q + 5]), pack_bf16x2(f[8 * q + 6], f[8 * q + 7]));
            if (s == 3)
              reinterpret_cast<float2*>(lf.stats_out)[((long long)grow * num_n_tiles + n_blk) * Cfg::EPI_GROUPS + half] =
                  make_float2(st_mean, st_m2);
          }
#pragma unroll
          for (int q = 0; q < 8; ++q) {
            const int phys = q ^ (erow & 7);
            *reinterpret_cast<float4*>(cd_row + phys * 16) = make_float4(f[4 * q], f[4 * q + 1], f[4 * q + 2], f[4 * q + 3]);
          }
          fence_proxy_async_smem();
          named_bar_sync(bar_id, 128);
          if (t == 0) {
            const int c0 = n0 + s * 32, r0 = m0 + cwg * 64;
            tma_store_2d(&tm_c, smem_cd_wg, c0, r0);
            tma_store_2d(&tm_c, smem_cd_wg + 64 * 128, c0 + 128, r0);
            tma_store_commit();
          }
        }
      }
    }
    if (t == 0) tma_store_wait_all<0>();
  }

  if (kCtaGroup == 2) cluster_sync_all();
}

typedef CUresult (*PFN_tmapEncodeTiled)(CUtensorMap*, CUtensorMapDataType, cuuint32_t, void*, const cuuint64_t*,
                                        const cuuint64_t*, const cuuint32_t*, const cuuint32_t*,
                                        CUtensorMapInterleave, CUtensorMapSwizzle, CUtensorMapL2promotion,
                                        CUtensorMapFloatOOBfill);

static PFN_tmapEncodeTiled get_encode_fn() {
  static PFN_tmapEncodeTiled fn = nullptr;
  if (!fn) {
    void* p = nullptr;
    cudaDriverEntryPointQueryResult q;
    if (cudaGetDriverEntryPoint("cuTensorMapEncodeTiled", &p, cudaEnableDefault, &q) != cudaSuccess ||
        q != cudaDriverEntryPointSuccess || !p) {
      set_last_error("cuTensorMapEncodeTiled driver entry point not available");
      return nullptr;
    }
    fn = reinterpret_cast<PFN_tmapEncodeTiled>(p);
  }
  return fn;
}

int make_tmap_2d(CUtensorMap* out, const void* ptr, int elem_bytes, long long rows, long long cols, long long ld,
                 int box_rows, int box_cols) {
  PFN_tmapEncodeTiled enc = get_encode_fn();
  if (!enc) return -3;
  CUtensorMapDataType dt = (elem_bytes == 2) ? CU_TENSOR_MAP_DATA_TYPE_BFLOAT16 : CU_TENSOR_MAP_DATA_TYPE_FLOAT32;
  cuuint64_t dims[2] = {(cuuint64_t)cols, (cuuint64_t)rows};
  cuuint64_t strides[1] = {(cuuint64_t)ld * (cuuint64_t)elem_bytes};
  cuuint32_t box[2] = {(cuuint32_t)box_cols, (cuuint32_t)box_rows};
  cuuint32_t estr[2] = {1, 1};
  if (box_cols * elem_bytes != 128) {
    set_last_error("make_tmap_2d: inner box must span 128 bytes");
    return -1;
  }
  CUresult r = enc(out, dt, 2, const_cast<void*>(ptr), dims, strides, box, estr, CU_TENSOR_MAP_INTERLEAVE_NONE,
                   CU_TENSOR_MAP_SWIZZLE_128B, CU_TENSOR_MAP_L2_PROMOTION_L2_256B,
                   CU_TENSOR_MAP_FLOAT_OOB_FILL_NONE);
  if (r != CUDA_SUCCESS) {
    set_last_error("cuTensorMapEncodeTiled failed with CUresult %d (rows=%lld cols=%lld ld=%lld elem=%d)", (int)r,
                   rows, cols, ld, elem_bytes);
    return -3;
  }
  return 0;
}

template <int kCtaGroup, int kEpi, typename OutT>
static int launch_inst(const CUtensorMap& ta, const CUtensorMap& tb, const CUtensorMap& tc, const float* bias,
                       const void* residual, long long ldr, int M, int N, int K, int num_sms, cudaStream_t stream,
                       float* cand_val = nullptr, int* cand_idx = nullptr, float* lse_part = nullptr,
                       int n_chunks = 1, const LnFold& lf = LnFold(), const ColFilter& cf = ColFilter(), int k_splits = 1,
                       int* splitk_flags = nullptr) {
  using Cfg = GemmCfg<kCtaGroup, kEpi>;
  auto kern = gemm_bf16_wgmma_kernel<kCtaGroup, kEpi, OutT>;
  static bool attr_set[64] = {};
  if (first_use_on_device(attr_set)) {
    SB_CUDA_CHECK(cudaFuncSetAttribute(kern, cudaFuncAttributeMaxDynamicSharedMemorySize, Cfg::SMEM_BYTES));
  }
  const int tile_m = Cfg::BLOCK_M * kCtaGroup;
  const long long num_m_tiles = (M + tile_m - 1) / tile_m;
  const long long num_tiles = num_m_tiles * ((N + Cfg::BLOCK_N - 1) / Cfg::BLOCK_N);
  long long clusters = num_sms / kCtaGroup;
  if (clusters > num_tiles * k_splits) clusters = num_tiles * k_splits;
  if (kEpi == EPI_TOPK && clusters > num_m_tiles * n_chunks) clusters = num_m_tiles * n_chunks;
  if (clusters < 1) clusters = 1;
  cudaLaunchConfig_t cfg = {};
  cfg.gridDim = dim3((unsigned)(clusters * kCtaGroup), 1, 1);
  cfg.blockDim = dim3(Cfg::THREADS, 1, 1);
  cfg.dynamicSmemBytes = Cfg::SMEM_BYTES;
  cfg.stream = stream;
  cudaLaunchAttribute attr[1];
  attr[0].id = cudaLaunchAttributeClusterDimension;
  attr[0].val.clusterDim.x = kCtaGroup;
  attr[0].val.clusterDim.y = 1;
  attr[0].val.clusterDim.z = 1;
  cfg.attrs = attr;
  cfg.numAttrs = 1;
  if (kCtaGroup == 2) {
    int max_clusters = 0;
    SB_CUDA_CHECK(cudaOccupancyMaxActiveClusters(&max_clusters, kern, &cfg));
    if (max_clusters < 1) {
      set_last_error("gemm_bf16: no 2-CTA cluster of the GEMM kernel fits on this device");
      return -2;
    }
    if (clusters > max_clusters) cfg.gridDim.x = (unsigned)(max_clusters * kCtaGroup);
  }
  SB_CUDA_CHECK(cudaLaunchKernelEx(&cfg, kern, ta, tb, tc, bias, reinterpret_cast<const OutT*>(residual), ldr, M, N, K,
                                   cand_val, cand_idx, lse_part, n_chunks, lf, cf, k_splits, splitk_flags));
  return 0;
}

int gemm_topk_chunks(int M, int N, int cta_group, int num_sms) {
  const int cg = (cta_group == 1) ? 1 : 2;
  const int clusters = (num_sms > 0 ? num_sms : device_sm_count()) / cg;
  const int num_m_tiles = (M + 128 * cg - 1) / (128 * cg);
  const int num_n_tiles = (N + 255) / 256;
  int want = clusters / num_m_tiles;
  if (want < 1) want = 1;
  if (want > num_n_tiles) want = num_n_tiles;
  const int tpc = (num_n_tiles + want - 1) / want;
  return (num_n_tiles + tpc - 1) / tpc;
}

int gemm_bf16_topk(const __nv_bfloat16* A, long long lda, const __nv_bfloat16* W, long long ldw, int M, int N, int K,
                   float* cand_val, int* cand_idx, float* lse_part, int n_chunks, int cta_group, int num_sms,
                   cudaStream_t stream, const ColFilter& cf) {
  if (M <= 0 || N <= 0) return 0;
  if (cf.thr != nullptr && (!cf.thr8 || !cf.cnt || !cf.buf || cf.cap <= 0)) {
    set_last_error("gemm_bf16_topk: column filter needs cnt, buf and a positive capacity");
    return -1;
  }
  if (K % 64 != 0 || K <= 0) {
    set_last_error("gemm_bf16_topk: K must be a positive multiple of 64 (got %d)", K);
    return -1;
  }
  const int num_n_tiles = (N + 255) / 256;
  if (n_chunks < 1 || n_chunks > num_n_tiles ||
      ((num_n_tiles + n_chunks - 1) / n_chunks) * (n_chunks - 1) >= num_n_tiles) {
    set_last_error("gemm_bf16_topk: invalid n_chunks=%d for %d n-tiles", n_chunks, num_n_tiles);
    return -1;
  }
  const int cg = (cta_group == 1) ? 1 : 2;
  CUtensorMap ta, tb;
  int rc;
  if ((rc = make_tmap_2d(&ta, A, 2, M, K, lda, 128, 64))) return rc;
  if ((rc = make_tmap_2d(&tb, W, 2, N, K, ldw, 256 / cg, 64))) return rc;
  const int sms = num_sms > 0 ? num_sms : device_sm_count();
  if (cg == 2)
    return launch_inst<2, EPI_TOPK, float>(ta, tb, ta , nullptr, nullptr, 0, M, N, K, sms, stream, cand_val,
                                           cand_idx, lse_part, n_chunks, LnFold(), cf);
  return launch_inst<1, EPI_TOPK, float>(ta, tb, ta , nullptr, nullptr, 0, M, N, K, sms, stream, cand_val,
                                         cand_idx, lse_part, n_chunks, LnFold(), cf);
}

int gemm_bf16(const GemmArgs& g, cudaStream_t stream) {
  if (g.M <= 0) return 0;
  if (g.allow_skinny && gemm_skinny_eligible(g) && !g.lf.stats_in && g.epi != EPI_BIAS_RESIDUAL_STATS)
    return gemm_skinny(g, stream);
  if (g.N % 256 != 0 || g.K % 64 != 0 || g.K <= 0 || g.N <= 0) {
    set_last_error("gemm_bf16: need N %% 256 == 0 and K %% 64 == 0 (got M=%d N=%d K=%d)", g.M, g.N, g.K);
    return -1;
  }
  if (g.epi == EPI_BIAS_RESIDUAL && !g.residual) {
    set_last_error("gemm_bf16: residual epilogue without residual pointer");
    return -1;
  }
  if (!g.bias) {
    set_last_error("gemm_bf16: bias pointer is required");
    return -1;
  }
  const int cg = (g.cta_group == 1) ? 1 : 2;
  const int out_bytes = g.out_fp32 ? 4 : 2;
  CUtensorMap ta, tb, tc;
  int rc;
  if ((rc = make_tmap_2d(&ta, g.A, 2, g.M, g.K, g.lda, 128, 64))) return rc;
  if ((rc = make_tmap_2d(&tb, g.W, 2, g.N, g.K, g.ldw, 256 / cg, 64))) return rc;
  if ((rc = make_tmap_2d(&tc, g.C, out_bytes, g.M, g.N, g.ldc, 64, 128 / out_bytes))) return rc;
  const int sms = g.num_sms > 0 ? g.num_sms : device_sm_count();
  int epi = g.epi;
  if (epi == EPI_BIAS_RESIDUAL && g.out_fp32 && g.residual == g.C && g.ldr == g.ldc) epi = EPI_BIAS_ACCUM;
  if (epi == EPI_BIAS_ACCUM && !g.out_fp32) {
    set_last_error("gemm_bf16: accumulate epilogue needs fp32 output");
    return -1;
  }

  if (g.lf.stats_in != nullptr) {
    if ((epi != EPI_BIAS && epi != EPI_BIAS_RELU) || !g.lf.colsum || g.lf.chunks < 1 || g.lf.chunks > 8 ||
        g.K != kLnPartCols * g.lf.chunks) {
      set_last_error("gemm_bf16: folded LayerNorm input needs a bias / bias+ReLU epilogue and K = 128 * chunks <= 1024 "
                     "(K=%d chunks=%d)", g.K, g.lf.chunks);
      return -1;
    }
  }
  if (epi == EPI_BIAS_RESIDUAL_STATS) {
    if (!g.out_fp32 || !g.residual || !g.lf.h_out || !g.lf.stats_out || g.lf.ldh < g.N) {
      set_last_error("gemm_bf16: the residual+statistics epilogue needs fp32 C, a residual, h_out and stats_out");
      return -1;
    }
  } else if (g.lf.h_out != nullptr || g.lf.stats_out != nullptr) {
    set_last_error("gemm_bf16: h_out / stats_out are outputs of EPI_BIAS_RESIDUAL_STATS only");
    return -1;
  }

  if (epi == EPI_BIAS_ACCUM && cg == 2 && g.splitk_flags != nullptr) {
    const long long tiles = (long long)((g.M + 255) / 256) * (g.N / 256);
    const long long clusters = sms / 2;
    const int num_kb = g.K / 64;
    int best = 1;
    double best_cost = 1e30;
    for (int ks = 1; ks <= 4; ++ks) {
      if (num_kb / ks < 8) break;
      const double cost = double((tiles * ks + clusters - 1) / clusters) * (double(num_kb) / ks + 8.0);
      if (cost < best_cost * 0.95) { best_cost = cost; best = ks; }
    }
    if (best > 1 && tiles * 2 * 2 <= g.splitk_flags_len)
      return launch_inst<2, EPI_BIAS_ACCUM, float>(ta, tb, tc, g.bias, g.residual, g.ldr, g.M, g.N, g.K, sms, stream, nullptr,
                                                   nullptr, nullptr, 1, LnFold(), ColFilter(), best, g.splitk_flags);
  }

#define SB_DISPATCH(CG, EPI, T)                                                                                   \
  return launch_inst<CG, EPI, T>(ta, tb, tc, g.bias, g.residual, g.ldr, g.M, g.N, g.K, sms, stream, nullptr, nullptr, \
                                 nullptr, 1, g.lf)
#define SB_DISPATCH_EPI(CG, T)                                              \
  switch (epi) {                                                            \
    case EPI_BIAS: SB_DISPATCH(CG, EPI_BIAS, T);                            \
    case EPI_BIAS_RELU: SB_DISPATCH(CG, EPI_BIAS_RELU, T);                  \
    case EPI_BIAS_SILU: SB_DISPATCH(CG, EPI_BIAS_SILU, T);                  \
    case EPI_BIAS_TANH: SB_DISPATCH(CG, EPI_BIAS_TANH, T);                  \
    case EPI_BIAS_RESIDUAL: SB_DISPATCH(CG, EPI_BIAS_RESIDUAL, T);          \
    case EPI_BIAS_ACCUM: SB_DISPATCH(CG, EPI_BIAS_ACCUM, float);            \
    case EPI_BIAS_RESIDUAL_STATS: SB_DISPATCH(CG, EPI_BIAS_RESIDUAL_STATS, float); \
    default: set_last_error("gemm_bf16: bad epilogue %d", epi); return -1;  \
  }
  if (cg == 2) {
    if (g.out_fp32) { SB_DISPATCH_EPI(2, float) } else { SB_DISPATCH_EPI(2, __nv_bfloat16) }
  } else {
    if (g.out_fp32) { SB_DISPATCH_EPI(1, float) } else { SB_DISPATCH_EPI(1, __nv_bfloat16) }
  }
#undef SB_DISPATCH
#undef SB_DISPATCH_EPI
  return -1;
}

}
```

sonar_b200/csrc/sonar_b200_internal.h:

```cpp
#pragma once

#include "../../include/sonar_b200.h"

#include <cuda.h>
#include <cuda_bf16.h>
#include <cuda_runtime.h>
#include <stdint.h>
#include <string.h>

#include <vector>

namespace sb {

enum EpiMode { EPI_BIAS = 0, EPI_BIAS_RELU = 1, EPI_BIAS_RESIDUAL = 2, EPI_BIAS_ACCUM = 3, EPI_TOPK = 4, EPI_BIAS_SILU = 5,
               EPI_BIAS_RESIDUAL_STATS = 6, EPI_BIAS_TANH = 7 };
constexpr int kTopkCandidates = 16;
enum PoolMode { POOL_MAX = 1, POOL_MEAN = 2, POOL_LAST = 3 };

void set_last_error(const char* fmt, ...);

int require_hopper(const char* who, int* num_sms);

template <class Weights>
bool has_null_pointer(const Weights& w) {
  static_assert(sizeof(Weights) % sizeof(void*) == 0, "a weight struct holds pointers only");
  for (size_t i = 0; i < sizeof(Weights) / sizeof(void*); ++i) {
    const void* p;
    memcpy(&p, reinterpret_cast<const char*>(&w) + i * sizeof(void*), sizeof(void*));
    if (!p) return true;
  }
  return false;
}

constexpr size_t kWorkspaceAlign = 1024;

inline size_t align_up(size_t v, size_t a) { return (v + a - 1) / a * a; }

struct Carver {
  uintptr_t base;
  size_t off = 0;
  explicit Carver(void* p) : base(reinterpret_cast<uintptr_t>(p)) {}
  template <class T>
  T* take(size_t bytes, size_t align = kWorkspaceAlign) {
    T* p = reinterpret_cast<T*>(base + off);
    off = align_up(off + bytes, align);
    return p;
  }
};

inline void* workspace_base(void* workspace) {
  return reinterpret_cast<void*>((reinterpret_cast<uintptr_t>(workspace) + kWorkspaceAlign - 1) &
                                 ~uintptr_t(kWorkspaceAlign - 1));
}

template <class Layout, class Carve>
int bind_workspace(const char* who, void* workspace, size_t workspace_bytes, Layout* ws, Carve&& carve) {
  void* base = workspace_base(workspace);
  *ws = carve(base);
  const size_t need = (reinterpret_cast<uintptr_t>(base) - reinterpret_cast<uintptr_t>(workspace)) + ws->bytes;
  if (need > workspace_bytes) {
    set_last_error("%s: workspace too small (%zu bytes given, %zu needed)", who, workspace_bytes, need);
    return SB_ERR_INVALID;
  }
  return SB_OK;
}

inline bool first_use_on_device(bool (&flags)[64]) {
  int dev = 0;
  if (cudaGetDevice(&dev) != cudaSuccess || dev < 0 || dev >= 64) return true;
  if (flags[dev]) return false;
  flags[dev] = true;
  return true;
}

constexpr int kLnPartCols = 128;
struct LnFold {
  const float* stats_in = nullptr;
  const float* colsum = nullptr;
  int chunks = 0;
  float eps = 0.f;
  __nv_bfloat16* h_out = nullptr;
  long long ldh = 0;
  float* stats_out = nullptr;
};

inline int device_sm_count() {
  int dev = 0, n = 0;
  if (cudaGetDevice(&dev) != cudaSuccess || cudaDeviceGetAttribute(&n, cudaDevAttrMultiProcessorCount, dev) != cudaSuccess || n < 1)
    return 1;
  return n;
}

struct GemmArgs {
  const __nv_bfloat16* A = nullptr;
  long long lda = 0;
  const __nv_bfloat16* W = nullptr;
  long long ldw = 0;
  void* C = nullptr;
  long long ldc = 0;
  int out_fp32 = 0;
  const float* bias = nullptr;
  const void* residual = nullptr;
  long long ldr = 0;
  int M = 0, N = 0, K = 0;
  int epi = EPI_BIAS;
  int cta_group = 2;
  int num_sms = 0;
  LnFold lf;
  int allow_skinny = 0;
  int* splitk_flags = nullptr;
  long long splitk_flags_len = 0;
};

inline GemmArgs gemm_args(const void* A, long long lda, const void* W, long long ldw, void* C, long long ldc, int out_fp32,
                          const float* bias, int M, int N, int K, int epi, int num_sms) {
  GemmArgs g;
  g.A = static_cast<const __nv_bfloat16*>(A); g.lda = lda;
  g.W = static_cast<const __nv_bfloat16*>(W); g.ldw = ldw;
  g.C = C; g.ldc = ldc; g.out_fp32 = out_fp32; g.bias = bias;
  if (epi == EPI_BIAS_RESIDUAL || epi == EPI_BIAS_RESIDUAL_STATS) { g.residual = C; g.ldr = ldc; }
  g.M = M; g.N = N; g.K = K; g.epi = epi;
  g.num_sms = num_sms;
  return g;
}

int gemm_bf16(const GemmArgs& g, cudaStream_t stream);

bool gemm_skinny_eligible(const GemmArgs& g);
int gemm_skinny(const GemmArgs& g, cudaStream_t stream);

struct ColFilter {
  float* thr = nullptr;
  const float* thr8 = nullptr;
  int* cnt = nullptr;
  uint2* buf = nullptr;
  int cap = 0;
};

int gemm_topk_chunks(int M, int N, int cta_group, int num_sms);
constexpr int kTopkListsPerChunk = 2;
inline int gemm_topk_lists(int n_chunks) { return kTopkListsPerChunk * n_chunks; }
int gemm_bf16_topk(const __nv_bfloat16* A, long long lda, const __nv_bfloat16* W, long long ldw, int M, int N, int K,
                   float* cand_val, int* cand_idx, float* lse_part, int n_chunks, int cta_group, int num_sms,
                   cudaStream_t stream, const ColFilter& cf = ColFilter());

int make_tmap_2d(CUtensorMap* out, const void* ptr, int elem_bytes, long long rows, long long cols, long long ld,
                 int box_rows, int box_cols);

int embed_tokens(const int64_t* ids, long long ids_stride, const int32_t* cu_seqlens, int B, int S,
                 const __nv_bfloat16* embed, long long vocab, const float* pos_table, int pos_rows, int D, float scale,
                 float* x, int* err_flag, cudaStream_t stream, int pos_offset = 0, __nv_bfloat16* h_out = nullptr,
                 float* stats_out = nullptr);

int fold_layernorm_weights(const __nv_bfloat16* W, const float* bias, const float* gamma, const float* beta, int N, int K,
                           __nv_bfloat16* Wf, float* colsum, float* bias_f, cudaStream_t stream);

int layernorm_bf16(const float* x, const float* gamma, const float* beta, float eps, __nv_bfloat16* y, long long T,
                   int D, cudaStream_t stream);

int layernorm_dual(const float* x, const float* gamma, const float* beta, float eps, float* y32, __nv_bfloat16* y16,
                   long long T, int D, cudaStream_t stream);

int attention_packed(const __nv_bfloat16* qkv, const int32_t* cu_seqlens, int B, int H, long long total_tokens, int num_sms,
                     __nv_bfloat16* out, cudaStream_t stream);

constexpr int kRelposTcMaxBatch = 2047;
int attention_relpos_tc(const __nv_bfloat16* qkv, const __nv_bfloat16* p, const float* u_bias, const float* v_bias,
                        const int32_t* cu_seqlens, int B, int H, long long total_tokens, int Npad, int S_center,
                        __nv_bfloat16* qu, __nv_bfloat16* qv, __nv_bfloat16* out, int num_sms, cudaStream_t stream);

int broadcast_rows(const float* v, float* x, __nv_bfloat16* xb, int B, int D, cudaStream_t stream);

int pool_latent_attention(const __nv_bfloat16* qt, const __nv_bfloat16* mem, const int32_t* cu_seqlens, int B, int Hd, int D,
                          __nv_bfloat16* u, cudaStream_t stream);

struct AttentionPooler {
  struct Layer {
    SbPoolerLayerWeights w;
    __nv_bfloat16* wqk = nullptr;
    float* bqk = nullptr;
    __nv_bfloat16* wvo = nullptr;
    float* bvo = nullptr;
  };
  struct Ws {
    float* px = nullptr;
    __nv_bfloat16* ph = nullptr;
    __nv_bfloat16* pt = nullptr;
    __nv_bfloat16* qt = nullptr;
    __nv_bfloat16* u = nullptr;
  };
  std::vector<Layer> layers;
  void* absorbed = nullptr;
  const float* q0 = nullptr;
  const void* proj_w = nullptr;
  const float* proj_b = nullptr;
  int D = 0, E = 0, F = 0;
  float eps = 0.f;
  int num_sms = 0, cta_group = 2, allow_skinny = 0;

  int create(const char* who, const SbPoolerLayerWeights* w, int num_layers, const float* q0, const void* proj_w,
             const float* proj_b, int D, int E, int F, float eps, int num_sms, int cta_group, int allow_skinny);
  void destroy();
  Ws take(Carver& c, size_t B) const;
  int forward(const Ws& w, const __nv_bfloat16* mem, const int32_t* cu_seqlens, int B, float* out, cudaStream_t stream) const;
};

int ln_pool(const float* x, const int32_t* cu_seqlens, int B, int D, const float* gamma, const float* beta,
            float eps, int apply_ln, int pool_mode, float* out, float* encoded_padded, int S_padded,
            cudaStream_t stream);

}
```

sonar_b200/ops.py:

```python

from __future__ import annotations

from typing import Optional

import torch
from torch import Tensor

from . import _lib
from .speech_encoder import relpos_rows

POOLING_MODES = {"max": _lib.SB_POOL_MAX, "mean": _lib.SB_POOL_MEAN, "last": _lib.SB_POOL_LAST}


def _need_cuda(*tensors: Optional[Tensor]) -> None:
    for t in tensors:
        if t is not None and not t.is_cuda:
            raise RuntimeError("sonar_b200 runs on CUDA tensors only (no CPU fallback exists)")


def _stream() -> int:
    return torch.cuda.current_stream().cuda_stream


def _ptr(t: Optional[Tensor]) -> Optional[int]:
    return None if t is None else t.data_ptr()


def gemm_bf16(a: Tensor, w: Tensor, bias: Tensor, *, epilogue: str = "bias", residual: Optional[Tensor] = None,
              out_dtype: torch.dtype = torch.bfloat16, out: Optional[Tensor] = None, cta_group: int = 2) -> Tensor:
    _need_cuda(a, w, bias, residual, out)
    assert a.dtype == torch.bfloat16 and w.dtype == torch.bfloat16 and bias.dtype == torch.float32
    assert a.dim() == 2 and w.dim() == 2 and a.stride(1) == 1 and w.stride(1) == 1
    m, k = a.shape
    n = w.shape[0]
    assert w.shape[1] == k and bias.numel() == n
    epi = {"bias": _lib.SB_EPI_BIAS, "relu": _lib.SB_EPI_BIAS_RELU, "residual": _lib.SB_EPI_BIAS_RESIDUAL, "silu": 5,
           "tanh": _lib.SB_EPI_BIAS_TANH}[epilogue]
    if out is None:
        out = torch.empty((m, n), dtype=out_dtype, device=a.device)
    assert out.dtype in (torch.bfloat16, torch.float32) and out.stride(1) == 1
    if epilogue == "residual":
        assert residual is not None and residual.dtype == out.dtype and residual.stride(1) == 1
    rc = _lib.load().sb_gemm_bf16(
        a.data_ptr(), a.stride(0), w.data_ptr(), w.stride(0), out.data_ptr(), out.stride(0),
        1 if out.dtype == torch.float32 else 0, bias.data_ptr(), _ptr(residual),
        residual.stride(0) if residual is not None else 0, m, n, k, epi, cta_group, _stream())
    _lib.check(rc, "sb_gemm_bf16")
    return out


def layernorm(x: Tensor, gamma: Tensor, beta: Tensor, eps: float = 1e-5) -> Tensor:
    _need_cuda(x, gamma, beta)
    assert x.dtype == torch.float32 and x.is_contiguous() and x.dim() == 2
    y = torch.empty(x.shape, dtype=torch.bfloat16, device=x.device)
    rc = _lib.load().sb_layernorm(x.data_ptr(), gamma.data_ptr(), beta.data_ptr(), eps, y.data_ptr(),
                                  x.shape[0], x.shape[1], _stream())
    _lib.check(rc, "sb_layernorm")
    return y


def cu_seqlens_of(seq_lens) -> Tensor:
    lens = torch.as_tensor(seq_lens, dtype=torch.int64).cpu()
    cu = torch.zeros(lens.numel() + 1, dtype=torch.int32)
    cu[1:] = torch.cumsum(lens, 0).to(torch.int32)
    return cu


def fold_layernorm(w: Tensor, bias: Tensor, gamma: Tensor, beta: Tensor):
    _need_cuda(w, bias, gamma, beta)
    assert w.dtype == torch.bfloat16 and w.is_contiguous()
    n, k = w.shape
    wf = torch.empty_like(w)
    colsum = torch.empty((n,), dtype=torch.float32, device=w.device)
    bias_f = torch.empty((n,), dtype=torch.float32, device=w.device)
    rc = _lib.load().sb_fold_layernorm(w.data_ptr(), bias.data_ptr(), gamma.data_ptr(), beta.data_ptr(), n, k, wf.data_ptr(),
                                       colsum.data_ptr(), bias_f.data_ptr(), _stream())
    _lib.check(rc, "sb_fold_layernorm")
    return wf, colsum, bias_f


def gemm_residual_stats(a: Tensor, w: Tensor, bias: Tensor, x: Tensor):
    _need_cuda(a, w, bias, x)
    m, k = a.shape
    n = w.shape[0]
    assert x.shape == (m, n) and x.dtype == torch.float32 and x.is_contiguous() and n % 256 == 0
    h = torch.empty((m, n), dtype=torch.bfloat16, device=a.device)
    stats = torch.empty((m, n // 128, 2), dtype=torch.float32, device=a.device)
    rc = _lib.load().sb_gemm_residual_stats(a.data_ptr(), a.stride(0), w.data_ptr(), w.stride(0), x.data_ptr(), n,
                                            bias.data_ptr(), h.data_ptr(), n, stats.data_ptr(), m, n, k, _stream())
    _lib.check(rc, "sb_gemm_residual_stats")
    return h, stats


def gemm_residual_splitk(a: Tensor, w: Tensor, bias: Tensor, x: Tensor, counters: Tensor) -> Tensor:
    _need_cuda(a, w, bias, x, counters)
    m, k = a.shape
    n = w.shape[0]
    assert x.shape == (m, n) and x.dtype == torch.float32 and x.is_contiguous() and counters.dtype == torch.int32
    rc = _lib.load().sb_gemm_residual_splitk(a.data_ptr(), a.stride(0), w.data_ptr(), w.stride(0), x.data_ptr(), n,
                                             bias.data_ptr(), m, n, k, counters.data_ptr(), counters.numel(), _stream())
    _lib.check(rc, "sb_gemm_residual_splitk")
    return x


def gemm_ln_consumer(a: Tensor, wf: Tensor, bias_f: Tensor, colsum: Tensor, stats: Tensor, eps: float = 1e-5,
                     relu: bool = False) -> Tensor:
    _need_cuda(a, wf, bias_f, colsum, stats)
    m, k = a.shape
    n = wf.shape[0]
    out = torch.empty((m, n), dtype=torch.bfloat16, device=a.device)
    rc = _lib.load().sb_gemm_ln_consumer(a.data_ptr(), a.stride(0), wf.data_ptr(), wf.stride(0), out.data_ptr(), n,
                                         bias_f.data_ptr(), colsum.data_ptr(), stats.data_ptr(), eps, m, n, k,
                                         1 if relu else 0, _stream())
    _lib.check(rc, "sb_gemm_ln_consumer")
    return out


def attention(qkv: Tensor, cu_seqlens: Tensor, num_heads: int) -> Tensor:
    _need_cuda(qkv, cu_seqlens)
    assert qkv.dtype == torch.bfloat16 and qkv.is_contiguous() and cu_seqlens.dtype == torch.int32
    t = qkv.shape[0]
    d = 64 * num_heads
    assert qkv.shape[1] == 3 * d
    out = torch.empty((t, d), dtype=torch.bfloat16, device=qkv.device)
    rc = _lib.load().sb_attention(qkv.data_ptr(), cu_seqlens.data_ptr(), cu_seqlens.numel() - 1, num_heads, t,
                                  out.data_ptr(), _stream())
    _lib.check(rc, "sb_attention")
    return out


def embed(ids: Tensor, cu_seqlens: Tensor, table: Tensor, pos_table: Tensor, scale: float, total_tokens: int) -> Tensor:
    _need_cuda(ids, cu_seqlens, table, pos_table)
    assert ids.dtype == torch.int64 and ids.stride(1) == 1 and table.dtype == torch.bfloat16
    b, s = ids.shape
    d = table.shape[1]
    x = torch.empty((total_tokens, d), dtype=torch.float32, device=ids.device)
    err = torch.zeros(1, dtype=torch.int32, device=ids.device)
    rc = _lib.load().sb_embed(ids.data_ptr(), ids.stride(0), cu_seqlens.data_ptr(), b, s, table.data_ptr(),
                              table.shape[0], pos_table.data_ptr(), pos_table.shape[0], d, scale, x.data_ptr(),
                              err.data_ptr(), _stream())
    _lib.check(rc, "sb_embed")
    if int(err.item()) != 0:
        raise ValueError("sb_embed: token id outside [0, vocab_size)")
    return x


def pool_packed(x: Tensor, cu_seqlens: Tensor, pooling: str, *, gamma: Optional[Tensor] = None,
                beta: Optional[Tensor] = None, eps: float = 1e-5, encoded_seq_len: int = 0):
    _need_cuda(x, cu_seqlens, gamma, beta)
    assert x.dtype == torch.float32 and x.is_contiguous()
    b = cu_seqlens.numel() - 1
    d = x.shape[1]
    out = torch.empty((b, d), dtype=torch.float32, device=x.device)
    enc = torch.empty((b, encoded_seq_len, d), dtype=torch.float32, device=x.device) if encoded_seq_len > 0 else None
    rc = _lib.load().sb_pool(x.data_ptr(), cu_seqlens.data_ptr(), b, d, _ptr(gamma), _ptr(beta), eps,
                             1 if gamma is not None else 0, POOLING_MODES[pooling.lower()], out.data_ptr(),
                             _ptr(enc), encoded_seq_len, _stream())
    _lib.check(rc, "sb_pool")
    return (out, enc) if enc is not None else out


def pool_latent_attention(qt: Tensor, mem: Tensor, cu_seqlens: Tensor) -> Tensor:
    _need_cuda(qt, mem, cu_seqlens)
    assert qt.dtype == torch.bfloat16 and mem.dtype == torch.bfloat16 and cu_seqlens.dtype == torch.int32
    assert qt.is_contiguous() and mem.is_contiguous() and qt.dim() == 3 and mem.dim() == 2
    b, hd, d = qt.shape
    assert mem.shape[1] == d and cu_seqlens.numel() == b + 1
    u = torch.empty_like(qt)
    rc = _lib.load().sb_pool_latent_attention(qt.data_ptr(), mem.data_ptr(), cu_seqlens.data_ptr(), b, hd, d,
                                              u.data_ptr(), _stream())
    _lib.check(rc, "sb_pool_latent_attention")
    return u


RELPOS_IMPLS = {"wgmma": 0, "mma_sync": 1}


def _out_rows(out: Optional[Tensor], t: int, d: int, device) -> Tensor:
    if out is None:
        return torch.empty((t, d), dtype=torch.bfloat16, device=device)
    assert out.dtype == torch.bfloat16 and out.shape == (t, d) and out.is_contiguous()
    return out


def attention_relpos(qkv: Tensor, p: Tensor, u_bias: Tensor, v_bias: Tensor, cu_seqlens: Tensor, num_heads: int, *,
                     impl: str = "wgmma", out: Optional[Tensor] = None) -> Tensor:
    _need_cuda(qkv, p, u_bias, v_bias, cu_seqlens, out)
    d = 64 * num_heads
    t = qkv.shape[0]
    assert qkv.dtype == torch.bfloat16 and qkv.is_contiguous() and qkv.shape == (t, 3 * d)
    assert u_bias.dtype == torch.float32 and v_bias.dtype == torch.float32 and u_bias.numel() == v_bias.numel() == d
    assert cu_seqlens.dtype == torch.int32
    s_center = int(cu_seqlens.cpu().diff().max())
    npad = relpos_rows(s_center)
    assert p.dtype == torch.bfloat16 and p.is_contiguous() and p.shape == (npad, d), (tuple(p.shape), npad)
    out = _out_rows(out, t, d, qkv.device)
    code = RELPOS_IMPLS[impl]
    qu = qv = vp = None
    if code == 0:
        qu = torch.empty((t, d), dtype=torch.bfloat16, device=qkv.device)
        qv = torch.empty_like(qu)
    else:
        vp = torch.empty((num_heads, npad), dtype=torch.float32, device=qkv.device)
    rc = _lib.load().sb_attention_relpos(qkv.data_ptr(), p.data_ptr(), u_bias.data_ptr(), v_bias.data_ptr(),
                                         cu_seqlens.data_ptr(), cu_seqlens.numel() - 1, num_heads, t, npad, s_center, code,
                                         _ptr(qu), _ptr(qv), _ptr(vp), out.data_ptr(), _stream())
    _lib.check(rc, "sb_attention_relpos")
    return out


def conformer_conv(g: Tensor, cu_seqlens: Tensor, dw: Tensor, bn_scale: Tensor, bn_shift: Tensor, *,
                   out: Optional[Tensor] = None) -> Tensor:
    _need_cuda(g, cu_seqlens, dw, bn_scale, bn_shift, out)
    t, d2 = g.shape
    d = d2 // 2
    assert g.dtype == torch.bfloat16 and g.is_contiguous() and cu_seqlens.dtype == torch.int32
    assert dw.dtype == torch.float32 and dw.is_contiguous() and dw.shape == (d, 31)
    assert bn_scale.dtype == bn_shift.dtype == torch.float32 and bn_scale.numel() == bn_shift.numel() == d
    max_len = int(cu_seqlens.cpu().diff().max())
    out = _out_rows(out, t, d, g.device)
    rc = _lib.load().sb_conformer_conv(g.data_ptr(), cu_seqlens.data_ptr(), cu_seqlens.numel() - 1, max_len, d, dw.data_ptr(),
                                       bn_scale.data_ptr(), bn_shift.data_ptr(), out.data_ptr(), _stream())
    _lib.check(rc, "sb_conformer_conv")
    return out


def speech_frontend(fbank: Tensor, cu_seqlens: Tensor, gamma: Tensor, beta: Tensor, eps: float = 1e-5, *,
                    out: Optional[Tensor] = None) -> Tensor:
    _need_cuda(fbank, cu_seqlens, gamma, beta, out)
    assert fbank.dtype == torch.float32 and fbank.is_contiguous() and fbank.dim() == 3 and fbank.shape[2] == 80
    assert gamma.dtype == beta.dtype == torch.float32 and gamma.numel() == beta.numel() == 160
    assert cu_seqlens.dtype == torch.int32 and cu_seqlens.numel() == fbank.shape[0] + 1
    cu = cu_seqlens.cpu()
    max_len, t = int(cu.diff().max()), int(cu[-1])
    out = _out_rows(out, t, 192, fbank.device)
    rc = _lib.load().sb_speech_frontend(fbank.data_ptr(), fbank.shape[1], cu_seqlens.data_ptr(), fbank.shape[0], max_len,
                                        gamma.data_ptr(), beta.data_ptr(), eps, out.data_ptr(), _stream())
    _lib.check(rc, "sb_speech_frontend")
    return out


LSTM_TILE_ROWS = 64


def lstm_gate_rows(hidden_size: int = 512, num_dirs: int = 1) -> Tensor:
    n = torch.arange(4 * hidden_size)
    one = (n % 128) // 32 * hidden_size + n // 128 * 32 + n % 32
    return torch.cat([one + d * 4 * hidden_size for d in range(num_dirs)])


def lstm_recurrent(g: Tensor, w_hh: Tensor, cu_seqlens: Tensor, tile_seqs: Tensor, num_dirs: int, *,
                   pool: bool = False, pad_mask: Optional[Tensor] = None, tail_keep: Optional[Tensor] = None,
                   padding_value: float = 0.0) -> Tensor:
    _need_cuda(g, w_hh, cu_seqlens, tile_seqs, pad_mask, tail_keep)
    assert g.dtype == torch.bfloat16 and w_hh.dtype == torch.bfloat16 and g.stride(1) == 1 and w_hh.is_contiguous()
    assert cu_seqlens.dtype == torch.int32 and tile_seqs.dtype == torch.int32 and tile_seqs.numel() % LSTM_TILE_ROWS == 0
    h = w_hh.shape[1]
    assert w_hh.shape[0] == num_dirs * 4 * h and g.shape[1] >= num_dirs * 4 * h
    for m in (pad_mask, tail_keep):
        assert m is None or m.dtype == torch.uint8
    t, b = g.shape[0], cu_seqlens.numel() - 1
    if pool:
        out = torch.empty((b, num_dirs * h), dtype=torch.float32, device=g.device)
        y, pool_out, ld = None, out, out.stride(0)
    else:
        out = torch.empty((t, num_dirs * h), dtype=torch.bfloat16, device=g.device)
        y, pool_out, ld = out, None, out.stride(0)
    rc = _lib.load().sb_lstm_recurrent(g.data_ptr(), g.stride(0), w_hh.data_ptr(), cu_seqlens.data_ptr(), tile_seqs.data_ptr(),
                                       tile_seqs.numel() // LSTM_TILE_ROWS, num_dirs, _ptr(y), ld, _ptr(pool_out), ld,
                                       _ptr(pad_mask), _ptr(tail_keep), padding_value, _stream())
    _lib.check(rc, "sb_lstm_recurrent")
    return out


def blaser_featurize(src: Tensor, mt: Tensor, ref: Optional[Tensor], input_form: str, *, normalize: bool = False,
                     out_dtype: torch.dtype = torch.float32) -> Tensor:
    _need_cuda(src, mt, ref)
    qe = {"COMET": False, "QE": True}[input_form]
    for t in (src, mt) + (() if qe else (ref,)):
        assert t.dtype == torch.float32 and t.is_contiguous() and t.shape == src.shape and t.dim() == 2
    n, e = src.shape
    out = torch.empty((n, (4 if qe else 6) * e), dtype=out_dtype, device=src.device)
    rc = _lib.load().sb_blaser_featurize(src.data_ptr(), mt.data_ptr(), None if qe else ref.data_ptr(), e, n, e,
                                         _lib.SB_BLASER_QE if qe else _lib.SB_BLASER_COMET, int(normalize),
                                         out.data_ptr(), int(out_dtype == torch.float32), _stream())
    _lib.check(rc, "sb_blaser_featurize")
    return out
```

Before: 4437.

## Add ping-pong GEMM schedule with 4-CTA clusters and L2 prefetch for accumulate epilogue

Adds a ping-pong variant of the WGMMA GEMM in which the two consumer warpgroups take alternate tiles of 64 rows. Named barriers hand the MMA turn from one warpgroup to the other, so one warpgroup's epilogue overlaps the other's mainloop. The variant runs on 4-CTA clusters that multicast B. Auto mode enables it for the fp32 accumulate (residual) epilogue when K<=1024 and there are enough tiles. The accumulate path also issues an L2 prefetch of the output tile near the end of the K loop, so the TMA reduce-add finds its data in L2. Risks are smaller M tiles per warpgroup, larger clusters that may not schedule well, and more template instances.

```diff
diff --git a/include/sonar_b200.h b/include/sonar_b200.h
--- a/include/sonar_b200.h
+++ b/include/sonar_b200.h
@@ -24,6 +24,10 @@
 #define SB_EPI_BIAS_RESIDUAL 2
 #define SB_EPI_BIAS_SILU 5
 #define SB_EPI_BIAS_TANH 7
+
+#define SB_GEMM_SCHEDULE_AUTO 0
+#define SB_GEMM_SCHEDULE_COOPERATIVE 1
+#define SB_GEMM_SCHEDULE_PINGPONG 2
 
 typedef struct SbEncoder SbEncoder;
 
@@ -107,7 +111,7 @@
 
 int sb_gemm_bf16(const void* A, int64_t lda, const void* W, int64_t ldw, void* C, int64_t ldc, int32_t out_fp32,
                  const float* bias, const void* residual, int64_t ldr, int32_t M, int32_t N, int32_t K, int32_t epi,
-                 int32_t cta_group, void* stream);
+                 int32_t cta_group, int32_t schedule, void* stream);
 
 int sb_layernorm(const float* x, const float* gamma, const float* beta, float eps, void* y, int64_t T, int32_t D,
                  void* stream);
diff --git a/sonar_b200/_lib.py b/sonar_b200/_lib.py
--- a/sonar_b200/_lib.py
+++ b/sonar_b200/_lib.py
@@ -10,6 +10,7 @@
 
 SB_POOL_MAX, SB_POOL_MEAN, SB_POOL_LAST, SB_POOL_ATTENTION = 1, 2, 3, 4
 SB_EPI_BIAS, SB_EPI_BIAS_RELU, SB_EPI_BIAS_RESIDUAL, SB_EPI_BIAS_TANH = 0, 1, 2, 7
+SB_GEMM_SCHEDULE_AUTO, SB_GEMM_SCHEDULE_COOPERATIVE, SB_GEMM_SCHEDULE_PINGPONG = 0, 1, 2
 SB_BLASER_COMET, SB_BLASER_QE = 0, 1
 SB_ERR_INVALID, SB_ERR_CUDA, SB_ERR_DRIVER, SB_ERR_INPUT = -1, -2, -3, -4
 
@@ -120,7 +121,7 @@
     "sb_encoder_check_inputs": (C.c_int, [C.c_void_p, C.c_void_p, C.c_void_p]),
     "sb_gemm_bf16": (C.c_int, [C.c_void_p, C.c_int64, C.c_void_p, C.c_int64, C.c_void_p, C.c_int64,
                                C.c_int32, C.c_void_p, C.c_void_p, C.c_int64, C.c_int32, C.c_int32,
-                               C.c_int32, C.c_int32, C.c_int32, C.c_void_p]),
+                               C.c_int32, C.c_int32, C.c_int32, C.c_int32, C.c_void_p]),
     "sb_layernorm": (C.c_int, [C.c_void_p, C.c_void_p, C.c_void_p, C.c_float, C.c_void_p, C.c_int64,
                                C.c_int32, C.c_void_p]),
     "sb_attention": (C.c_int, [C.c_void_p, C.c_void_p, C.c_int32, C.c_int32, C.c_int64, C.c_void_p, C.c_void_p]),
diff --git a/sonar_b200/csrc/common.cuh b/sonar_b200/csrc/common.cuh
--- a/sonar_b200/csrc/common.cuh
+++ b/sonar_b200/csrc/common.cuh
@@ -57,6 +57,10 @@
   asm volatile("bar.sync %0, %1;" ::"r"(id), "r"(nthreads) : "memory");
 }
 
+__device__ __forceinline__ void named_bar_arrive(uint32_t id, uint32_t nthreads) {
+  asm volatile("bar.arrive %0, %1;" ::"r"(id), "r"(nthreads) : "memory");
+}
+
 __device__ __forceinline__ void mbar_init(uint64_t* bar, uint32_t count) {
   asm volatile("mbarrier.init.shared::cta.b64 [%0], %1;" ::"r"(smem_u32(bar)), "r"(count) : "memory");
 }
@@ -126,6 +130,12 @@
 
 __device__ __forceinline__ void tma_prefetch_desc(const CUtensorMap* m) {
   asm volatile("prefetch.tensormap [%0];" ::"l"(reinterpret_cast<uint64_t>(m)) : "memory");
+}
+
+__device__ __forceinline__ void tma_prefetch_l2_2d(const CUtensorMap* m, int c0, int c1) {
+  asm volatile("cp.async.bulk.prefetch.tensor.2d.L2.global.tile [%0, {%1, %2}];" ::"l"(reinterpret_cast<uint64_t>(m)),
+               "r"(c0), "r"(c1)
+               : "memory");
 }
 
 __device__ __forceinline__ void tma_load_2d(void* smem_dst, const CUtensorMap* m, uint64_t* bar, int c0,
diff --git a/sonar_b200/csrc/encoder.cu b/sonar_b200/csrc/encoder.cu
--- a/sonar_b200/csrc/encoder.cu
+++ b/sonar_b200/csrc/encoder.cu
@@ -400,7 +400,7 @@
 
 int sb_gemm_bf16(const void* A, int64_t lda, const void* W, int64_t ldw, void* C, int64_t ldc, int32_t out_fp32,
                  const float* bias, const void* residual, int64_t ldr, int32_t M, int32_t N, int32_t K, int32_t epi,
-                 int32_t cta_group, void* stream) {
+                 int32_t cta_group, int32_t schedule, void* stream) {
   if (!A || !W || !C) { set_last_error("sb_gemm_bf16: null pointer"); return SB_ERR_INVALID; }
   int sms = 0;
   if (int rc = require_hopper("sb_gemm_bf16", &sms)) return rc;
@@ -408,6 +408,7 @@
   g.residual = residual; g.ldr = ldr;
   g.cta_group = cta_group == 1 ? 1 : 2;
   g.allow_skinny = (cta_group == 0);
+  g.schedule = schedule;
   return gemm_bf16(g, reinterpret_cast<cudaStream_t>(stream));
 }
 
diff --git a/sonar_b200/csrc/gemm_wgmma.cu b/sonar_b200/csrc/gemm_wgmma.cu
--- a/sonar_b200/csrc/gemm_wgmma.cu
+++ b/sonar_b200/csrc/gemm_wgmma.cu
@@ -8,10 +8,11 @@
 
 constexpr bool epi_row_wise(int epi) { return epi == EPI_BIAS_RESIDUAL_STATS || epi == EPI_TOPK; }
 
-template <int kCtaGroup, int kEpi>
+template <int kCtaGroup, int kEpi, bool kPingPong>
 struct GemmCfg {
   static constexpr bool ROW_WISE = epi_row_wise(kEpi);
-  static constexpr int BLOCK_M = 128;
+  static_assert(!(kPingPong && ROW_WISE), "the row-wise epilogues are cooperative only");
+  static constexpr int BLOCK_M = kPingPong ? 64 : 128;
   static constexpr int BLOCK_N = 256;
   static constexpr int BLOCK_K = 64;
   static constexpr int LOAD_N = BLOCK_N / kCtaGroup;
@@ -19,7 +20,7 @@
   static constexpr int B_BYTES = BLOCK_N * BLOCK_K * 2;
   static constexpr int STAGES = ROW_WISE ? 3 : 4;
   static constexpr int EPI_GROUPS = 2;
-  static constexpr int CD_BYTES = 2 * 64 * 128;
+  static constexpr int CD_BYTES = (kPingPong ? 4 : 2) * 64 * 128;
   static constexpr int TRANS_LD = 68;
   static constexpr int TRANS_BYTES = ROW_WISE ? 64 * TRANS_LD * 4 : 0;
   static constexpr int LN_BYTES = 64 * 8;
@@ -87,15 +88,18 @@
 }
 
 
-template <int kCtaGroup, int kEpi, typename OutT>
-__global__ void __launch_bounds__(GemmCfg<kCtaGroup, kEpi>::THREADS, 1)
+constexpr int kAccumPrefetchKb = 6;
+
+template <int kCtaGroup, int kEpi, typename OutT, bool kPingPong>
+__global__ void __launch_bounds__(GemmCfg<kCtaGroup, kEpi, kPingPong>::THREADS, 1)
 gemm_bf16_wgmma_kernel(const __grid_constant__ CUtensorMap tm_a, const __grid_constant__ CUtensorMap tm_b,
                        const __grid_constant__ CUtensorMap tm_c, const float* __restrict__ bias,
                        const OutT* residual, long long ldr, int M, int N, int K, float* __restrict__ cand_val,
                        int* __restrict__ cand_idx, float* __restrict__ lse_part, int n_chunks, const LnFold lf,
                        const ColFilter cf, int k_splits, int* __restrict__ splitk_flags) {
   constexpr bool kSweep = (kEpi == EPI_TOPK);
-  using Cfg = GemmCfg<kCtaGroup, kEpi>;
+  constexpr bool kSplitK = (kEpi == EPI_BIAS_ACCUM) && !kPingPong;
+  using Cfg = GemmCfg<kCtaGroup, kEpi, kPingPong>;
   extern __shared__ uint8_t smem_raw[];
   uint8_t* smem = reinterpret_cast<uint8_t*>((reinterpret_cast<uintptr_t>(smem_raw) + 1023) & ~uintptr_t(1023));
   uint8_t* smem_a = smem;
@@ -109,7 +113,7 @@
   const int warp_idx = threadIdx.x >> 5;
   const int lane = threadIdx.x & 31;
   const int wg_idx = __shfl_sync(0xffffffffu, threadIdx.x >> 7, 0);
-  const uint32_t cta_rank = (kCtaGroup == 2) ? cluster_ctarank() : 0u;
+  const uint32_t cta_rank = (kCtaGroup > 1) ? cluster_ctarank() : 0u;
 
   if (threadIdx.x == 0) {
     tma_prefetch_desc(&tm_a);
@@ -117,11 +121,11 @@
     tma_prefetch_desc(&tm_c);
     for (int i = 0; i < Cfg::STAGES; ++i) {
       mbar_init(&full_bar[i], 1);
-      mbar_init(&empty_bar[i], 8 * kCtaGroup);
+      mbar_init(&empty_bar[i], (kPingPong ? 4 : 8) * kCtaGroup);
     }
     fence_mbar_init();
   }
-  if (kCtaGroup == 2) cluster_sync_all(); else __syncthreads();
+  if (kCtaGroup > 1) cluster_sync_all(); else __syncthreads();
 
   const int tile_m = Cfg::BLOCK_M * kCtaGroup;
   const int num_m_tiles = (M + tile_m - 1) / tile_m;
@@ -130,9 +134,9 @@
   const int cluster_id = blockIdx.x / kCtaGroup;
   const int num_clusters = gridDim.x / kCtaGroup;
   TileSched<kSweep> sched{num_m_tiles, num_n_tiles, cluster_id, num_clusters, n_chunks,
-                          (num_n_tiles + n_chunks - 1) / n_chunks, (kEpi == EPI_BIAS_ACCUM) ? k_splits : 1};
-  auto kb_begin = [&](int split) { return (kEpi == EPI_BIAS_ACCUM && k_splits > 1) ? split * num_kb / k_splits : 0; };
-  auto kb_end = [&](int split) { return (kEpi == EPI_BIAS_ACCUM && k_splits > 1) ? (split + 1) * num_kb / k_splits : num_kb; };
+                          (num_n_tiles + n_chunks - 1) / n_chunks, kSplitK ? k_splits : 1};
+  auto kb_begin = [&](int split) { return (kSplitK && k_splits > 1) ? split * num_kb / k_splits : 0; };
+  auto kb_end = [&](int split) { return (kSplitK && k_splits > 1) ? (split + 1) * num_kb / k_splits : num_kb; };
   int m_blk, n_blk, chunk;
   bool first_in_item, last_in_item;
 
@@ -144,13 +148,21 @@
       while (sched.next(m_blk, n_blk, chunk, first_in_item, last_in_item)) {
         const int m0 = m_blk * tile_m + int(cta_rank) * Cfg::BLOCK_M;
         const int n0 = n_blk * Cfg::BLOCK_N + int(cta_rank) * Cfg::LOAD_N;
-        const int kb1 = kb_end(chunk);
-        for (int kb = kb_begin(chunk); kb < kb1; ++kb) {
+        const int kb0 = kb_begin(chunk), kb1 = kb_end(chunk);
+        [[maybe_unused]] const int kb_pf = max(kb0, kb1 - kAccumPrefetchKb);
+        for (int kb = kb0; kb < kb1; ++kb) {
+          if constexpr (kEpi == EPI_BIAS_ACCUM) {
+            if (kb == kb_pf) {
+              for (int r = 0; r < Cfg::BLOCK_M; r += 64)
+                for (int c = 0; c < Cfg::BLOCK_N; c += 32) tma_prefetch_l2_2d(&tm_c, n_blk * Cfg::BLOCK_N + c, m0 + r);
+            }
+          }
           mbar_wait(&empty_bar[stage], phase ^ 1);
           mbar_arrive_expect_tx(&full_bar[stage], Cfg::A_BYTES + Cfg::B_BYTES);
           tma_load_2d(smem_a + stage * Cfg::A_BYTES, &tm_a, &full_bar[stage], kb * Cfg::BLOCK_K, m0);
           uint8_t* b_dst = smem_b + stage * Cfg::B_BYTES + int(cta_rank) * (Cfg::LOAD_N * Cfg::BLOCK_K * 2);
-          if (kCtaGroup == 2) tma_load_2d_multicast(b_dst, &tm_b, &full_bar[stage], kb * Cfg::BLOCK_K, n0, 0x3);
+          if (kCtaGroup > 1)
+            tma_load_2d_multicast(b_dst, &tm_b, &full_bar[stage], kb * Cfg::BLOCK_K, n0, (1u << kCtaGroup) - 1u);
           else tma_load_2d(b_dst, &tm_b, &full_bar[stage], kb * Cfg::BLOCK_K, n0);
           if (++stage == Cfg::STAGES) { stage = 0; phase ^= 1; }
         }
@@ -163,16 +175,19 @@
     const int t = threadIdx.x & 127;
     const int half = t >> 6;
     const int erow = t & 63;
-    const int row_in_tile = cwg * 64 + erow;
+    const int wg_row = kPingPong ? 0 : cwg * 64;
+    const int row_in_tile = wg_row + erow;
     const int frow = (warp_idx & 3) * 16 + (lane >> 2);
     uint8_t* smem_cd_wg = smem_cd + cwg * Cfg::CD_BYTES;
     float* trans = reinterpret_cast<float*>(smem_tr + cwg * Cfg::TRANS_BYTES);
     float2* ln_sm = reinterpret_cast<float2*>(smem_ln + cwg * Cfg::LN_BYTES);
     const uint32_t bar_id = 1 + cwg;
-    const uint64_t a_desc0 = wgmma_desc_kmajor_sw128(smem_u32(smem_a) + cwg * 64 * 128);
+    const uint32_t my_turn_bar = 3 + cwg, other_turn_bar = 4 - cwg;
+    int item_idx = 0;
+    const uint64_t a_desc0 = wgmma_desc_kmajor_sw128(smem_u32(smem_a) + wg_row * 128);
     const uint64_t b_desc0 = wgmma_desc_kmajor_sw128(smem_u32(smem_b));
     auto release = [&](int stage) {
-      if (kCtaGroup == 2) { if (lane < 2) mbar_arrive_cluster(&empty_bar[stage], lane); }
+      if (kCtaGroup > 1) { if (lane < kCtaGroup) mbar_arrive_cluster(&empty_bar[stage], lane); }
       else if (lane == 0) mbar_arrive(&empty_bar[stage]);
     };
     int stage = 0;
@@ -198,11 +213,27 @@
           if (i < lf.chunks) part_next[i] = sp[i];
       }
     };
-    if constexpr (kEpi == EPI_BIAS || kEpi == EPI_BIAS_RELU) {
+    if constexpr ((kEpi == EPI_BIAS || kEpi == EPI_BIAS_RELU) && !kPingPong) {
       fold_in = lf.stats_in != nullptr;
       if (fold_in) fetch_parts();
     }
     while (sched.next(m_blk, n_blk, chunk, first_in_item, last_in_item)) {
+      bool more_items = false;
+      if constexpr (kPingPong) {
+        const bool mine = (item_idx & 1) == cwg;
+        ++item_idx;
+        if (!mine) {
+          const int s = stage + num_kb;
+          phase ^= uint32_t(s / Cfg::STAGES) & 1u;
+          stage = s % Cfg::STAGES;
+          continue;
+        }
+        TileSched<kSweep> peek = sched;
+        int mb, nb, ch;
+        bool f0, f1;
+        more_items = peek.next(mb, nb, ch, f0, f1);
+        if (item_idx > 1) named_bar_sync(my_turn_bar, 256);
+      }
       const int m0 = m_blk * tile_m + int(cta_rank) * Cfg::BLOCK_M;
       const int n0 = n_blk * Cfg::BLOCK_N;
       const int grow = m0 + row_in_tile;
@@ -262,6 +293,9 @@
           prev = stage;
           if (++stage == Cfg::STAGES) { stage = 0; phase ^= 1; }
         }
+        if constexpr (kPingPong) {
+          if (more_items) named_bar_arrive(other_turn_bar, 256);
+        }
         wgmma_wait<0>();
         wgmma_fence_regs(acc);
         release(prev);
@@ -273,7 +307,7 @@
         constexpr int NBUF = Cfg::CD_BYTES / BOX_BYTES;
         static_assert(NBUF >= 2 && BOXES % NBUF == 0, "staging buffers must alternate the same way in every tile");
         const int fcol = 2 * (lane & 3);
-        const int grow_lo = m0 + cwg * 64 + frow, grow_hi = grow_lo + 8;
+        const int grow_lo = m0 + wg_row + frow, grow_hi = grow_lo + 8;
         if (fold_in) named_bar_sync(bar_id, 128);
         const bool with_bias = !(kEpi == EPI_BIAS_ACCUM && chunk > 0);
         auto epi = [&](float v, float b, float c, float2 ln, int grow, int col) -> float {
@@ -334,10 +368,10 @@
           if (t == 0) tma_store_wait_read<NBUF - 2>();
           named_bar_sync(bar_id, 128);
           if (t == 0) {
-            const int c0 = n0 + b * BOX_COLS, r0 = m0 + cwg * 64;
+            const int c0 = n0 + b * BOX_COLS, r0 = m0 + wg_row;
             if constexpr (kEpi == EPI_BIAS_ACCUM) {
               int* flag = nullptr;
-              if (k_splits > 1) {
+              if (kSplitK && k_splits > 1) {
                 flag = splitk_flags + ((long long)(m_blk * num_n_tiles + n_blk) * kCtaGroup + int(cta_rank)) * 2 + cwg;
                 if (b == 0 && chunk > 0) {
                   while (ld_acquire_gpu(flag) != chunk) __nanosleep(64);
@@ -346,7 +380,7 @@
               }
               tma_reduce_add_2d(&tm_c, reinterpret_cast<const void*>(smem_cd_wg + (b % NBUF) * BOX_BYTES), c0, r0);
               tma_store_commit();
-              if (k_splits > 1 && b == BOXES - 1) {
+              if (kSplitK && k_splits > 1 && b == BOXES - 1) {
                 tma_store_wait_all<0>();
                 fence_proxy_async_all();
                 __threadfence();
@@ -558,7 +592,7 @@
     if (t == 0) tma_store_wait_all<0>();
   }
 
-  if (kCtaGroup == 2) cluster_sync_all();
+  if (kCtaGroup > 1) cluster_sync_all();
 }
 
 typedef CUresult (*PFN_tmapEncodeTiled)(CUtensorMap*, CUtensorMapDataType, cuuint32_t, void*, const cuuint64_t*,
@@ -605,14 +639,14 @@
   return 0;
 }
 
-template <int kCtaGroup, int kEpi, typename OutT>
+template <int kCtaGroup, int kEpi, typename OutT, bool kPingPong = false>
 static int launch_inst(const CUtensorMap& ta, const CUtensorMap& tb, const CUtensorMap& tc, const float* bias,
                        const void* residual, long long ldr, int M, int N, int K, int num_sms, cudaStream_t stream,
                        float* cand_val = nullptr, int* cand_idx = nullptr, float* lse_part = nullptr,
                        int n_chunks = 1, const LnFold& lf = LnFold(), const ColFilter& cf = ColFilter(), int k_splits = 1,
                        int* splitk_flags = nullptr) {
-  using Cfg = GemmCfg<kCtaGroup, kEpi>;
-  auto kern = gemm_bf16_wgmma_kernel<kCtaGroup, kEpi, OutT>;
+  using Cfg = GemmCfg<kCtaGroup, kEpi, kPingPong>;
+  auto kern = gemm_bf16_wgmma_kernel<kCtaGroup, kEpi, OutT, kPingPong>;
   static bool attr_set[64] = {};
   if (first_use_on_device(attr_set)) {
     SB_CUDA_CHECK(cudaFuncSetAttribute(kern, cudaFuncAttributeMaxDynamicSharedMemorySize, Cfg::SMEM_BYTES));
@@ -636,11 +670,11 @@
   attr[0].val.clusterDim.z = 1;
   cfg.attrs = attr;
   cfg.numAttrs = 1;
-  if (kCtaGroup == 2) {
+  if (kCtaGroup > 1) {
     int max_clusters = 0;
     SB_CUDA_CHECK(cudaOccupancyMaxActiveClusters(&max_clusters, kern, &cfg));
     if (max_clusters < 1) {
-      set_last_error("gemm_bf16: no 2-CTA cluster of the GEMM kernel fits on this device");
+      set_last_error("gemm_bf16: no %d-CTA cluster of the GEMM kernel fits on this device", kCtaGroup);
       return -2;
     }
     if (clusters > max_clusters) cfg.gridDim.x = (unsigned)(max_clusters * kCtaGroup);
@@ -709,20 +743,36 @@
     set_last_error("gemm_bf16: bias pointer is required");
     return -1;
   }
+  if (g.schedule != SB_GEMM_SCHEDULE_AUTO && g.schedule != SB_GEMM_SCHEDULE_COOPERATIVE &&
+      g.schedule != SB_GEMM_SCHEDULE_PINGPONG) {
+    set_last_error("gemm_bf16: bad schedule %d", g.schedule);
+    return -1;
+  }
   const int cg = (g.cta_group == 1) ? 1 : 2;
   const int out_bytes = g.out_fp32 ? 4 : 2;
-  CUtensorMap ta, tb, tc;
-  int rc;
-  if ((rc = make_tmap_2d(&ta, g.A, 2, g.M, g.K, g.lda, 128, 64))) return rc;
-  if ((rc = make_tmap_2d(&tb, g.W, 2, g.N, g.K, g.ldw, 256 / cg, 64))) return rc;
-  if ((rc = make_tmap_2d(&tc, g.C, out_bytes, g.M, g.N, g.ldc, 64, 128 / out_bytes))) return rc;
-  const int sms = g.num_sms > 0 ? g.num_sms : device_sm_count();
   int epi = g.epi;
   if (epi == EPI_BIAS_RESIDUAL && g.out_fp32 && g.residual == g.C && g.ldr == g.ldc) epi = EPI_BIAS_ACCUM;
   if (epi == EPI_BIAS_ACCUM && !g.out_fp32) {
     set_last_error("gemm_bf16: accumulate epilogue needs fp32 output");
     return -1;
   }
+  const bool pingpong_ok = !epi_row_wise(epi) && g.lf.stats_in == nullptr && g.splitk_flags == nullptr && cg == 2;
+  if (g.schedule == SB_GEMM_SCHEDULE_PINGPONG && !pingpong_ok) {
+    set_last_error("gemm_bf16: the ping-pong schedule takes cta_group 2 and the column-wise epilogues without LayerNorm "
+                   "folding or split-K");
+    return -1;
+  }
+  const int sms = g.num_sms > 0 ? g.num_sms : device_sm_count();
+  const long long pp_items = (long long)((g.M + 255) / 256) * (g.N / 256);
+  const bool pingpong = pingpong_ok && (g.schedule == SB_GEMM_SCHEDULE_PINGPONG ||
+                                        (g.schedule == SB_GEMM_SCHEDULE_AUTO && epi == EPI_BIAS_ACCUM &&
+                                         g.K <= 1024 && pp_items >= 8LL * (sms / 4)));
+  const int cluster = pingpong ? 4 : cg;
+  CUtensorMap ta, tb, tc;
+  int rc;
+  if ((rc = make_tmap_2d(&ta, g.A, 2, g.M, g.K, g.lda, pingpong ? 64 : 128, 64))) return rc;
+  if ((rc = make_tmap_2d(&tb, g.W, 2, g.N, g.K, g.ldw, 256 / cluster, 64))) return rc;
+  if ((rc = make_tmap_2d(&tc, g.C, out_bytes, g.M, g.N, g.ldc, 64, 128 / out_bytes))) return rc;
 
   if (g.lf.stats_in != nullptr) {
     if ((epi != EPI_BIAS && epi != EPI_BIAS_RELU) || !g.lf.colsum || g.lf.chunks < 1 || g.lf.chunks > 8 ||
@@ -758,9 +808,11 @@
                                                    nullptr, nullptr, 1, LnFold(), ColFilter(), best, g.splitk_flags);
   }
 
-#define SB_DISPATCH(CG, EPI, T)                                                                                   \
-  return launch_inst<CG, EPI, T>(ta, tb, tc, g.bias, g.residual, g.ldr, g.M, g.N, g.K, sms, stream, nullptr, nullptr, \
-                                 nullptr, 1, g.lf)
+#define SB_DISPATCH_SCHED(CG, EPI, T, PP)                                                                             \
+  return launch_inst<CG, EPI, T, PP>(ta, tb, tc, g.bias, g.residual, g.ldr, g.M, g.N, g.K, sms, stream, nullptr, nullptr, \
+                                     nullptr, 1, g.lf)
+#define SB_DISPATCH(CG, EPI, T)                                   \
+  if (pingpong) { SB_DISPATCH_SCHED(4, EPI, T, true); } else { SB_DISPATCH_SCHED(CG, EPI, T, false); }
 #define SB_DISPATCH_EPI(CG, T)                                              \
   switch (epi) {                                                            \
     case EPI_BIAS: SB_DISPATCH(CG, EPI_BIAS, T);                            \
@@ -769,7 +821,7 @@
     case EPI_BIAS_TANH: SB_DISPATCH(CG, EPI_BIAS_TANH, T);                  \
     case EPI_BIAS_RESIDUAL: SB_DISPATCH(CG, EPI_BIAS_RESIDUAL, T);          \
     case EPI_BIAS_ACCUM: SB_DISPATCH(CG, EPI_BIAS_ACCUM, float);            \
-    case EPI_BIAS_RESIDUAL_STATS: SB_DISPATCH(CG, EPI_BIAS_RESIDUAL_STATS, float); \
+    case EPI_BIAS_RESIDUAL_STATS: SB_DISPATCH_SCHED(CG, EPI_BIAS_RESIDUAL_STATS, float, false); \
     default: set_last_error("gemm_bf16: bad epilogue %d", epi); return -1;  \
   }
   if (cg == 2) {
@@ -777,6 +829,7 @@
   } else {
     if (g.out_fp32) { SB_DISPATCH_EPI(1, float) } else { SB_DISPATCH_EPI(1, __nv_bfloat16) }
   }
+#undef SB_DISPATCH_SCHED
 #undef SB_DISPATCH
 #undef SB_DISPATCH_EPI
   return -1;
diff --git a/sonar_b200/csrc/sonar_b200_internal.h b/sonar_b200/csrc/sonar_b200_internal.h
--- a/sonar_b200/csrc/sonar_b200_internal.h
+++ b/sonar_b200/csrc/sonar_b200_internal.h
@@ -106,6 +106,7 @@
   int epi = EPI_BIAS;
   int cta_group = 2;
   int num_sms = 0;
+  int schedule = SB_GEMM_SCHEDULE_AUTO;
   LnFold lf;
   int allow_skinny = 0;
   int* splitk_flags = nullptr;
diff --git a/sonar_b200/ops.py b/sonar_b200/ops.py
--- a/sonar_b200/ops.py
+++ b/sonar_b200/ops.py
@@ -10,6 +10,8 @@
 from .speech_encoder import relpos_rows
 
 POOLING_MODES = {"max": _lib.SB_POOL_MAX, "mean": _lib.SB_POOL_MEAN, "last": _lib.SB_POOL_LAST}
+GEMM_SCHEDULES = {"auto": _lib.SB_GEMM_SCHEDULE_AUTO, "cooperative": _lib.SB_GEMM_SCHEDULE_COOPERATIVE,
+                  "pingpong": _lib.SB_GEMM_SCHEDULE_PINGPONG}
 
 
 def _need_cuda(*tensors: Optional[Tensor]) -> None:
@@ -27,7 +29,8 @@
 
 
 def gemm_bf16(a: Tensor, w: Tensor, bias: Tensor, *, epilogue: str = "bias", residual: Optional[Tensor] = None,
-              out_dtype: torch.dtype = torch.bfloat16, out: Optional[Tensor] = None, cta_group: int = 2) -> Tensor:
+              out_dtype: torch.dtype = torch.bfloat16, out: Optional[Tensor] = None, cta_group: int = 2,
+              schedule: str = "auto") -> Tensor:
     _need_cuda(a, w, bias, residual, out)
     assert a.dtype == torch.bfloat16 and w.dtype == torch.bfloat16 and bias.dtype == torch.float32
     assert a.dim() == 2 and w.dim() == 2 and a.stride(1) == 1 and w.stride(1) == 1
@@ -44,7 +47,7 @@
     rc = _lib.load().sb_gemm_bf16(
         a.data_ptr(), a.stride(0), w.data_ptr(), w.stride(0), out.data_ptr(), out.stride(0),
         1 if out.dtype == torch.float32 else 0, bias.data_ptr(), _ptr(residual),
-        residual.stride(0) if residual is not None else 0, m, n, k, epi, cta_group, _stream())
+        residual.stride(0) if residual is not None else 0, m, n, k, epi, cta_group, GEMM_SCHEDULES[schedule], _stream())
     _lib.check(rc, "sb_gemm_bf16")
     return out
 
```

Result: no change. 4436 (median of 6 runs) (-0.0%).
